# EPFL-VILAB/omnidata

Hardware: AMD Instinct MI355X
Metric: images/sec (384x384) DPT-Hybrid surface-normal inference (higher is better)
Workload: dtype bf16; 1 GPU; DPT-Hybrid-384 normal, batch 32/GPU, bf16, 1xMI355X (BASELINE.json configs[1]); batch_per_gpu=32, global_batch=32, parallelism=replicas x1 (no collective in the loop), ranks_seen=1, inflight=1

## Files before the change

### include/dptx.h

```cpp
#ifndef DPTX_H_
#define DPTX_H_

#include <stddef.h>
#include <stdint.h>

#ifdef __cplusplus
extern "C" {
#endif

typedef struct dptx_engine* dptx_handle;

enum {
  DPTX_OK = 0,
  DPTX_E_INVALID = -1,
  DPTX_E_KEY = -2,
  DPTX_E_HIP = -3,
  DPTX_E_NODEVICE = -4,
  DPTX_E_ALLOC = -5
};

enum { DPTX_DTYPE_BF16 = 0, DPTX_DTYPE_FP16 = 1, DPTX_DTYPE_BF16X3 = 2,
       DPTX_DTYPE_FP16X3 = 3, DPTX_DTYPE_MIXED = 4,
       DPTX_DTYPE_FP8 = 5 };
enum { DPTX_GROUP_RESNET = 1,
// ... 54 lines not shown
int dptx_forward_dual(dptx_handle h, const void* x_dev, int32_t x_dtype, void* y_normal_dev, void* y_depth_dev,
                      int32_t batch, int32_t height, int32_t width, void* stream);

int dptx_set_layer_precision(dptx_handle h, const char* conv_weight_key, int32_t mfmas);

int dptx_calibrate_fp8(dptx_handle h, const void* x_dev, int32_t x_dtype, void* y_dev, void* y2_dev,
                       int32_t batch, int32_t height, int32_t width, void* stream);
int dptx_fp8_get_calibration(dptx_handle h, float* scales, float* amax, int32_t capacity);
int dptx_fp8_set_calibration(dptx_handle h, const float* scales, int32_t n);

int dptx_range_status(dptx_handle h, int32_t* nonfinite, int32_t reset, void* stream);

int dptx_tap(dptx_handle h, const char* name, float* dst_host, size_t capacity_floats,
             int64_t shape4[4]);
int dptx_enable_taps(dptx_handle h, int on);

int dptx_forward_info(dptx_handle h, int64_t* launches, double* algorithmic_macs,
                      double* executed_macs);

int dptx_tune_schedule(dptx_handle h, const void* x_dev, int32_t x_dtype, void* y_dev, void* y_depth_dev, int32_t batch,
                       int32_t height, int32_t width, int32_t reps, void* stream);
int dptx_schedule_info(dptx_handle h, int32_t* split, int32_t* tuned, float* ms_single, float* ms_split);

int dptx_probe_stream_overlap(int32_t device_id, void* stream_a, void* stream_b, int32_t spin_us, float* ratio);

int dptx_set_profiling(dptx_handle h, int on);
int dptx_profile_get(dptx_handle h, int32_t category, double* ms, int64_t* launches,
                     double* macs_per_image);
int dptx_profile_dump(dptx_handle h, const char* path);

const char* dptx_last_error(dptx_handle h);
const char* dptx_version(void);

int dptx_preprocess_u8(const void* img_dev, int32_t H, int32_t W, int32_t C, int32_t row_stride_bytes,
                       int32_t depth_normalize, void* x_dev, void* stream);
int dptx_postprocess_normal_u8(const void* y_dev, void* rgb_u8_dev, void* stream);
int dptx_postprocess_depth(const void* y_dev, void* out512_dev, void* stream);
int dptx_resample_coeffs(int32_t in_size, int32_t out_size, int32_t* bounds, int32_t* kk, int32_t kk_capacity,
                         int32_t* ksize);

int dptx_refocus_workspace_bytes(int32_t B, int32_t C, int32_t H, int32_t W, int32_t n_quantiles, int64_t* bytes);
int dptx_refocus_quantiles(const float* depth, int32_t B, int32_t H, int32_t W, int32_t n_quantiles,
                           float* qvals , void* ws, int64_t ws_bytes, void* stream);
int dptx_refocus(const float* rgb, const float* depth, int32_t B, int32_t C, int32_t H, int32_t W, int32_t n_quantiles,
                 const float* qvals, const float* focus , const float* aperture ,
                 float* out, int64_t* segments , void* ws, int64_t ws_bytes, void* stream);

#define DPTX_MIDAS_SSI 1
#define DPTX_MIDAS_GRAD 2
#define DPTX_MIDAS_ALIGN 4
#define DPTX_MIDAS_INVERSE 8
#define DPTX_MIDAS_ALL 15
#define DPTX_MIDAS_RECORD_DOUBLES 32
#define DPTX_MIDAS_STATS 8
int dptx_midas_workspace_bytes(int32_t B, int32_t H, int32_t W, int32_t scales, int64_t* bytes);
int dptx_midas_loss(const float* pred, const float* target, const uint8_t* mask, int32_t B, int32_t H, int32_t W, int32_t terms,
                    int32_t scales, int32_t image_based, float alpha, float* losses, double* record , void* ws,
                    int64_t ws_bytes, void* stream);
int dptx_midas_loss_backward(const float* pred, const float* target, const uint8_t* mask, int32_t B, int32_t H, int32_t W,
                             int32_t terms, int32_t scales, int32_t image_based, float alpha, const double* record,
                             const float* grad_losses, float* grad_pred, void* stream);
int dptx_midas_stats(const float* pred, const float* target, const uint8_t* mask, int32_t B, int32_t H, int32_t W, int32_t terms,
                     float* stats, float* pred_aligned , float* target_aligned , void* ws,
                     int64_t ws_bytes, void* stream);

#define DPTX_VNL_RECORD_HEADER 64
int dptx_vnl_workspace_bytes(int32_t B, int32_t H, int32_t W, int32_t n, int64_t* bytes);
int dptx_vnl_prepare(const int32_t* p1, const int32_t* p2, const int32_t* p3, int32_t n, int32_t H, int32_t W, uint32_t* inverse,
                     void* ws, int64_t ws_bytes, void* stream);
int dptx_vnl_loss(const float* first, const float* second, int32_t B, int32_t H, int32_t W, float fx, float fy, float delta_z,
                  const int32_t* p1, const int32_t* p2, const int32_t* p3, int32_t n, int32_t select, float* loss_out,
                  uint8_t* record , void* ws, int64_t ws_bytes, void* stream);
int dptx_vnl_loss_backward(const float* first, const float* second, int32_t B, int32_t H, int32_t W, float fx, float fy,
                           const int32_t* p1, const int32_t* p2, const int32_t* p3, int32_t n, const uint8_t* record,
                           const uint32_t* inverse, const float* grad_out, float* grad_first ,
                           float* grad_second , void* stream);
int dptx_vnl_triples(const float* first, const float* second, int32_t B, int32_t H, int32_t W, float fx, float fy, float delta_z,
                     const int32_t* p1, const int32_t* p2, const int32_t* p3, int32_t n, uint8_t* keep, float* loss,
                     float* normals , void* stream);

#define DPTX_NORMAL_L1 1
#define DPTX_NORMAL_COS 2
#define DPTX_NORMAL_CLAMP_PRED 4
#define DPTX_NORMAL_RECORD_DOUBLES 1
int dptx_normal_workspace_bytes(int32_t B, int32_t H, int32_t W, int64_t* bytes);
int dptx_normal_loss(const float* pred, const float* target, const uint8_t* mask, int32_t B, int32_t H, int32_t W, int32_t flags,
                     float l1_weight, float* losses, double* record , void* ws, int64_t ws_bytes, void* stream);
int dptx_normal_loss_backward(const float* pred, const float* target, const uint8_t* mask, int32_t B, int32_t H, int32_t W,
                              int32_t flags, float l1_weight, const double* record, const float* grad_losses, float* grad_pred,
                              void* stream);
int dptx_normal_pixels(const float* pred, const float* target, const uint8_t* mask, int32_t B, int32_t H, int32_t W, int32_t flags,
                       float* cos , float* l1 , void* stream);
#define DPTX_MASKED_L1 0
#define DPTX_MASKED_MSE 1
#define DPTX_MASKED_VALUE 2
#define DPTX_MASKED_EMPTY_ZERO 4
int dptx_masked_workspace_bytes(int64_t n, int64_t* bytes);
int dptx_masked_loss(const float* pred, const float* target , const uint8_t* mask, int64_t n, int32_t kind,
                     float* loss, double* record , void* ws, int64_t ws_bytes, void* stream);
int dptx_masked_loss_backward(const float* pred, const float* target, const uint8_t* mask, int64_t n, int32_t kind,
                              const double* record, const float* grad_loss, float* grad_pred, void* stream);
int dptx_valid_mask(const float* mask_float, int32_t B, int32_t H, int32_t W, int32_t pool, uint8_t* valid, void* stream);

#define DPTX_EVAL_PER_IMAGE 1
#define DPTX_EVAL_NORMAL_FIELDS 9
#define DPTX_EVAL_DEPTH_FIELDS 8
int dptx_eval_workspace_bytes(int32_t B, int32_t H, int32_t W, int64_t* bytes);
int dptx_eval_normal(const float* pred, const float* target , const uint8_t* mask , int32_t B, int32_t H,
                     int32_t W, int32_t flags, double* out , void* ws, int64_t ws_bytes, void* stream);
int dptx_eval_depth(const float* pred, const float* target , const uint8_t* mask , int32_t B, int32_t H,
                    int32_t W, int32_t flags, double* out , void* ws, int64_t ws_bytes, void* stream);
int dptx_eval_normal_pixels(const float* pred, const float* target, int32_t B, int32_t H, int32_t W, double* ang, void* stream);


int dptx_op_set_planes(int64_t act_plane_elems, int64_t w_plane_elems);

int dptx_op_gemm(int32_t dtype, const void* A, const void* W, const float* bias, const void* R,
                 void* C, int32_t M, int32_t N, int32_t K, int32_t act, int32_t a_fp32,
                 int32_t c_fp32, int32_t r_fp32, void* stream);
int dptx_op_conv(int32_t dtype, const void* X, const void* Wt, const float* bias, const void* R,
                 void* Y, int32_t B, int32_t H, int32_t W, int32_t Cin, int32_t Cout,
                 int32_t ksize, int32_t stride, int32_t pad_t, int32_t pad_l, int32_t Ho,
                 int32_t Wo, int32_t a_relu, int32_t act, void* stream);
int dptx_op_conv_planes(int32_t dtype, const void* X, const void* Wt, const float* bias, const void* R, void* Y, int32_t B,
                        int32_t H, int32_t W, int32_t Cin, int32_t Cout, int32_t ksize, int32_t stride, int32_t pad_t,
                        int32_t pad_l, int32_t Ho, int32_t Wo, int32_t a_relu, int32_t act, int32_t epi2, int32_t c_hi_only,
                        int32_t r1_hi_only, void* stream);
int dptx_op_stem_conv(int32_t dtype, const float* x, const void* Wt, void* y, int32_t B, int32_t H, int32_t W,
                      void* stream);
int dptx_op_attention(int32_t dtype, const void* qkv, void* out, int32_t B, int32_t S,
                      int32_t heads, void* stream);
int dptx_op_layernorm(int32_t dtype, const float* x, const float* gamma, const float* beta,
                      void* y, int32_t M, int32_t C, float eps, void* stream);
int dptx_op_groupnorm(int32_t dtype, const void* X, const float* gamma, const float* beta,
                      const void* R, void* Y, int32_t B, int32_t HW, int32_t C, int32_t relu,
                      float eps, void* scratch_f32, void* stream);
int dptx_op_gn_relu_maxpool(int32_t dtype, const void* X, const float* gamma, const float* beta, void* Y, int32_t B,
                            int32_t H, int32_t W, int32_t C, float eps, void* scratch_f32, void* stream);
int dptx_op_cls_rows(int32_t dtype, const float* cls, const float* pos, float* X, int32_t B, int32_t S, int32_t C, void* X16,
                     float* row_stats, void* X8, float q_scale, void* stream);
int dptx_debug_set_trace(void* dev_buf);
int dptx_debug_arena_fill(dptx_handle h, int32_t byte_value);
int dptx_debug_arena_read(dptx_handle h, void* dst_host, size_t offset, size_t bytes);
int dptx_debug_arena_layout(dptx_handle h, char* dst, size_t capacity);
int dptx_debug_arena_checksums(dptx_handle h, void* out_dev, int32_t capacity, void* stream);
int dptx_debug_set_gemm_flags(int32_t flags);
int dptx_op_conv_fp8(const void* X8, const void* Wt8, const float* bias, const void* R, void* Y, void* Y8, int32_t B,
                     int32_t H, int32_t W, int32_t Cin, int32_t Cout, int32_t ksize, int32_t stride, int32_t pad_t,
                     int32_t pad_l, int32_t Ho, int32_t Wo, int32_t act, int32_t q_relu, float out_scale, void* stream);
int dptx_op_conv_groupnorm(int32_t dtype, const void* X, const void* Wt, void* Yraw, const float* gamma, const float* beta,
                           const void* R, void* Y, int32_t B, int32_t H, int32_t W, int32_t Cin, int32_t Cout,
                           int32_t ksize, int32_t stride, int32_t pad_t, int32_t pad_l, int32_t Ho, int32_t Wo,
                           int32_t relu, float eps, void* scratch_f32, void* stream);
int dptx_op_upsample2x(int32_t dtype, const void* X, void* Y, int32_t B, int32_t H, int32_t W,
                       int32_t C, void* stream);
int dptx_op_gemm_ln(int32_t dtype, const void* A, const void* W, const float* bias, void* C, int32_t M, int32_t N, int32_t K,
                    int32_t act, const float* ln_stats, const float* ln_colsum, int32_t ln_nblk, float ln_eps, void* stream);
int dptx_op_gemm_stream(int32_t dtype, const void* A, const void* W, const float* bias, void* C, float* row_stats, int32_t M,
                        int32_t N, int32_t K, void* stream);
int dptx_op_gemm_stream32(int32_t dtype, const void* A, const void* W, const float* bias, float* X, void* C16, float* row_stats,
                          int32_t M, int32_t N, int32_t K, void* stream);
int dptx_op_head_tail(int32_t dtype, const void* H0, const void* W2, const float* b2, const float* w4,
                      const float* b4, float* y, int32_t B, int32_t Hs, int32_t Ws, int32_t C,
                      int32_t relu_out, void* stream);

#ifdef __cplusplus
}
#endif
#endif
```

### omnidata_amd/build.py

```python
from __future__ import annotations

import os
import subprocess
import sys

HERE = os.path.dirname(os.path.abspath(__file__))
CSRC = os.path.join(HERE, "csrc")
LIB = os.path.join(HERE, "libdptx.so")
SOURCES = ["gemm.hip", "gemm_fp16.hip", "gemm_fp16e.hip", "gemm_x3.hip", "gemm_x2.hip", "gemm_fp8.hip", "attention.hip", "norm.hip", "misc.hip", "stem.hip", "head.hip", "prepost.hip", "refocus.hip", "midas_loss.hip", "vnl_loss.hip", "normal_loss.hip", "eval_metrics.hip", "engine.hip", "ops.hip"]
HEADERS = ["common.h", "kernels.h", "gemm_impl.h", "select.h", os.path.join("..", "..", "include", "dptx.h")]
_NOPK = ["-Xclang", "-target-feature", "-Xclang", "-packed-fp32-ops"]
SOURCE_FLAGS = {src: list(_NOPK) for src in ("norm.hip", "misc.hip", "gemm.hip", "gemm_fp16.hip", "gemm_fp16e.hip", "gemm_x3.hip",
                                             "gemm_x2.hip", "gemm_fp8.hip", "refocus.hip",
                                             "midas_loss.hip", "vnl_loss.hip", "normal_loss.hip", "eval_metrics.hip")}
EXPERIMENT_HEADERS = []


def source_hash(extra_flags=()) -> str:
    import hashlib
    h = hashlib.sha256()
    for name in sorted(SOURCES + HEADERS + EXPERIMENT_HEADERS):
        path = os.path.join(CSRC, name)
        h.update(os.path.basename(name).encode() + b"\0")
        with open(path, "rb") as f:
            h.update(f.read())
    h.update(" ".join(extra_flags).encode())
    h.update(repr(sorted(SOURCE_FLAGS.items())).encode())
    return h.hexdigest()[:16]


def _newer(dst: str, srcs) -> bool:
    if not os.path.exists(dst):
        return False
    t = os.path.getmtime(dst)
    return all(os.path.getmtime(s) <= t for s in srcs)


def built_hash(suffix: str = "") -> str:
    path = os.path.join(CSRC, "build" + suffix, "engine.srchash")
    return open(path).read().strip() if os.path.exists(path) else ""


def build(force: bool = False, verbose: bool = False) -> str:
    import fcntl
    suffix = os.environ.get("DPTX_LIB_SUFFIX", "")
    objdir = os.path.join(CSRC, "build" + suffix)
    os.makedirs(objdir, exist_ok=True)
    with open(os.path.join(objdir, ".lock"), "w") as lock:
        fcntl.flock(lock, fcntl.LOCK_EX)
        try:
            return _build_locked(force, verbose, suffix, objdir)
        finally:
            fcntl.flock(lock, fcntl.LOCK_UN)


def _build_locked(force: bool, verbose: bool, suffix: str, objdir: str) -> str:
    hipcc = os.environ.get("HIPCC", "/opt/rocm/bin/hipcc")
    extra = os.environ.get("DPTX_CXXFLAGS", "").split()
    LIB = os.path.join(HERE, f"libdptx{suffix}.so")
    hdrs = [os.path.join(CSRC, h) for h in HEADERS + EXPERIMENT_HEADERS]
    src_hash = source_hash(extra)
    hash_file = os.path.join(objdir, "engine.srchash")
    old_hash = open(hash_file).read().strip() if os.path.exists(hash_file) else ""
    objs = []
    procs = []
    for src in SOURCES:
        s = os.path.join(CSRC, src)
        o = os.path.join(objdir, src.replace(".hip", ".o"))
        objs.append(o)
        cmd = [hipcc, "--offload-arch=gfx950", "-O3", "-std=c++17", "-fPIC"] + SOURCE_FLAGS.get(src, []) + extra + ["-c", s, "-o", o]
        if src == "engine.hip":
            cmd.insert(-4, f'-DDPTX_SRC_HASH="{src_hash}"')
        cmd_file = o + ".cmd"
        same_cmd = os.path.exists(cmd_file) and open(cmd_file).read() == " ".join(cmd)
        if not force and same_cmd and _newer(o, [s] + hdrs):
            continue
        if verbose:
            print(" ".join(cmd))
        if os.path.exists(cmd_file):
            os.remove(cmd_file)
        procs.append((src, cmd_file, " ".join(cmd), subprocess.Popen(cmd, stdout=subprocess.PIPE, stderr=subprocess.STDOUT, text=True)))
    for src, cmd_file, cmd_txt, p in procs:
        out, _ = p.communicate()
        if p.returncode != 0:
            raise RuntimeError(f"hipcc failed on {src}:\n{out}")
        with open(cmd_file, "w") as f:
            f.write(cmd_txt)
    if force or procs or not _newer(LIB, objs):
        tmp = f"{LIB}.tmp{os.getpid()}"
        cmd = [hipcc, "--offload-arch=gfx950", "-shared", "-fPIC", "-o", tmp] + objs
        r = subprocess.run(cmd, stdout=subprocess.PIPE, stderr=subprocess.STDOUT, text=True)
        if r.returncode != 0:
            if os.path.exists(tmp):
                os.remove(tmp)
            raise RuntimeError(f"link failed:\n{r.stdout}")
        os.replace(tmp, LIB)
    with open(hash_file, "w") as f:
        f.write(src_hash + "\n")
    return LIB


if __name__ == "__main__":
    print(build(force="--force" in sys.argv, verbose=True))
```

### omnidata_amd/csrc/engine.hip

```cpp
#include <hip/hip_runtime.h>

#include <algorithm>
#include <cmath>
#include <cstdio>
#include <chrono>
#include <cstring>
#include <map>
#include <memory>
#include <string>
#include <unordered_map>
#include <vector>

#include "../../include/dptx.h"
#include "kernels.h"

using namespace dptx;

namespace {

constexpr int IMG = 384;
constexpr int S_TOK = 577;
constexpr int FEAT = 256;
const int STAGE_DEPTH[3] = {3, 4, 9};
const int STAGE_OUT[3] = {256, 512, 1024};
// ... 488 lines not shown
      const uint16_t hi = f32_to_fp16(x);
      d16[i] = hi;
      if (x3) d16[i + lo_elems] = f32_to_fp16(x - fp16_to_f32(hi));
      return;
    }
    const uint16_t hi = f32_to_bf16(x);
    d16[i] = hi;
    if (x3) d16[i + lo_elems] = f32_to_bf16(x - bf16_to_f32(hi));
  };
  auto r16 = [&](float x) { return bf ? bf16_to_f32(f32_to_bf16(x)) : fp16_to_f32(f32_to_fp16(x)); };
  for (const auto& s : e->spec) {
    if (s.role == R_UNUSED || s.role == R_DERIVED) continue;
    const std::vector<float>& src = e->staged.at(s.key);
    uint8_t* dst = e->host_blob.data() + e->packed_off.at(s.key);
    const bool fold_w = e->ln_fold && s.role == R_LINEAR && (ends_with(s.key, "attn.qkv.weight") || ends_with(s.key, "mlp.fc1.weight"));
    const bool fold_b = e->ln_fold && s.role == R_VEC && (ends_with(s.key, "attn.qkv.bias") || ends_with(s.key, "mlp.fc1.bias"));
    if (fold_w || fold_b) {
      const bool qkv = s.key.find("attn.qkv") != std::string::npos;
      const std::string blk = s.key.substr(0, s.key.find(qkv ? "attn.qkv" : "mlp.fc1"));
      const std::string wkey = blk + (qkv ? "attn.qkv.weight" : "mlp.fc1.weight");
      const std::vector<float>& W = e->staged.at(wkey);
      const std::vector<float>& gamma = e->staged.at(blk + (qkv ? "norm1.weight" : "norm2.weight"));
      const std::vector<float>& beta = e->staged.at(blk + (qkv ? "norm1.bias" : "norm2.bias"));
      const size_t K = gamma.size(), N = W.size() / K;
      if (fold_b) {
        float* d32 = (float*)dst;
        for (size_t n = 0; n < N; ++n) {
          double acc = src[n];
          for (size_t k = 0; k < K; ++k) acc += (double)W[n * K + k] * (double)beta[k];
          d32[n] = (float)acc;
        }
      } else {
        uint16_t* d16 = (uint16_t*)dst;
        float* cs = (float*)(e->host_blob.data() + e->packed_off.at(blk + (qkv ? "attn.qkv.lnsum" : "mlp.fc1.lnsum")));
        for (size_t n = 0; n < N; ++n) {
          double acc = 0.0;
          for (size_t k = 0; k < K; ++k) {
            const float wf = W[n * K + k] * gamma[k];
            put(d16, n * K + k, wf);
            acc += (double)r16(wf);
          }
          cs[n] = (float)acc;
        }
      }
      continue;
    }
    if (s.role == R_VEC || s.role == R_HEAD4) {
      memcpy(dst, src.data(), src.size() * 4);
      continue;
    }
    if (s.role == R_DECONV_BIAS) {
      for (int t = 0; t < 16; ++t) memcpy(dst + (size_t)t * src.size() * 4, src.data(), src.size() * 4);
      continue;
    }
    uint16_t* d16 = (uint16_t*)dst;
    if (s.role == R_LINEAR) {
      for (size_t i = 0; i < src.size(); ++i) put(d16, i, src[i]);
      continue;
    }
    if (s.role == R_DECONV) {
      const int CI = (int)s.shape[0], CO = (int)s.shape[1], K = (int)s.shape[2];
      for (int ci = 0; ci < CI; ++ci)
        for (int co = 0; co < CO; ++co)
          for (int dy = 0; dy < K; ++dy)
            for (int dx = 0; dx < K; ++dx)
              put(d16, ((size_t)(dy * K + dx) * CO + co) * CI + ci, src[(((size_t)ci * CO + co) * K + dy) * K + dx]);
      continue;
    }
    const int O = (int)s.shape[0], I = (int)s.shape[1], KH = (int)s.shape[2], KW = (int)s.shape[3];
    const size_t per_o = (size_t)I * KH * KW;
    const bool stem = (KH == 7);
    const size_t out_k = stem ? STEM_K : per_o;
    for (int o = 0; o < O; ++o) {
      const float* wo = src.data() + (size_t)o * per_o;
      double mean = 0.0, scale = 1.0;
      if (s.role == R_STDCONV) {
        double sum = 0.0;
        for (size_t i = 0; i < per_o; ++i) sum += wo[i];
        mean = sum / (double)per_o;
        double var = 0.0;
        for (size_t i = 0; i < per_o; ++i) { const double t = wo[i] - mean; var += t * t; }
        var /= (double)per_o;
        scale = e->cfg.ws_form == 0 ? 1.0 / (std::sqrt(var) + (double)e->cfg.ws_eps)
                                    : 1.0 / std::sqrt(var + (double)e->cfg.ws_eps);
      }
      for (int ky = 0; ky < KH; ++ky)
        for (int kx = 0; kx < KW; ++kx)
          for (int i = 0; i < I; ++i) {
            const double wv = ((double)wo[((size_t)i * KH + ky) * KW + kx] - mean) * scale;
            const size_t kidx = stem ? ((size_t)i * 7 + ky) * 8 + kx : ((size_t)ky * KW + kx) * I + i;
            put(d16, (size_t)o * out_k + kidx, (float)wv);
          }
    }
  }
  if (e->fp8()) {
    for (size_t si = 0; si < e->spec.size(); ++si) {
      const Spec& sp = e->spec[si];
      if (sp.role != R_CONV || !dptx_engine::fp8_weight(sp.key)) continue;
      const size_t off = e->packed_off.at(sp.key);
      const std::vector<float>& src = e->staged.at(sp.key);
      const int O = (int)sp.shape[0], I = (int)sp.shape[1], KH = (int)sp.shape[2], KW = (int)sp.shape[3];
      const size_t per_o = (size_t)I * KH * KW;
      uint8_t* d8 = e->host_blob.data() + e->packed_single + off / 2;
      float* inv = (float*)(e->host_blob.data() + e->packed_off.at(sp.key.substr(0, sp.key.size() - 6) + "f8scale"));
      for (int o = 0; o < O; ++o) {
        float mx = 0.f;
        for (size_t i = 0; i < per_o; ++i) mx = std::max(mx, std::fabs(src[(size_t)o * per_o + i]));
        const float sc = e4m3_channel_scale(mx, &inv[o]);
        for (int ky = 0; ky < KH; ++ky)
          for (int kx = 0; kx < KW; ++kx)
            for (int i = 0; i < I; ++i)
              d8[(size_t)o * per_o + ((size_t)ky * KW + kx) * I + i] = f32_to_e4m3(src[(((size_t)o * I + i) * KH + ky) * KW + kx] * sc);
      }
    }
  }
  if (e->fp8()) {
    for (size_t si = 0; si < e->spec.size(); ++si) {
      const Spec& sp = e->spec[si];
      if (sp.role != R_LINEAR || !dptx_engine::fp8_vit_weight(sp.key)) continue;
      const std::vector<float>& W = e->staged.at(sp.key);
      const size_t N = (size_t)sp.shape[0], K = (size_t)sp.shape[1];
      const bool fc2 = ends_with(sp.key, "mlp.fc2.weight"), qkv = ends_with(sp.key, "attn.qkv.weight");
      const std::string stem_key = sp.key.substr(0, sp.key.size() - 6);
      const std::string blk = sp.key.substr(0, sp.key.find(qkv ? "attn.qkv" : (fc2 ? "mlp.fc2" : "mlp.fc1")));
      const std::vector<float>* gamma = (!fc2 && e->ln_fold) ? &e->staged.at(blk + (qkv ? "norm1.weight" : "norm2.weight")) : nullptr;
      uint8_t* d8 = e->host_blob.data() + e->packed_single + e->packed_off.at(sp.key) / 2;
      float* inv = (float*)(e->host_blob.data() + e->packed_off.at(stem_key + "f8scale"));
      float* cs8 = fc2 ? nullptr : (float*)(e->host_blob.data() + e->packed_off.at(stem_key + "lnsum8"));
      for (size_t n = 0; n < N; ++n) {
        float mx = 0.f;
        for (size_t k = 0; k < K; ++k) mx = std::max(mx, std::fabs(W[n * K + k] * (gamma ? (*gamma)[k] : 1.0f)));
        const float sc = e4m3_channel_scale(mx, &inv[n]);
        double acc = 0.0;
        for (size_t k = 0; k < K; ++k) {
          const uint8_t q = f32_to_e4m3(W[n * K + k] * (gamma ? (*gamma)[k] : 1.0f) * sc);
          d8[n * K + k] = q;
          acc += (double)e4m3_to_f32(q);
        }
        if (cs8) cs8[n] = (float)(acc / (double)sc);
      }
    }
  }
  e->finalized = true;
  return DPTX_OK;
}

enum { LN_NONE = 0, LN_CONSUMER = 1, LN_PRODUCER = 2 };
struct GemmOpt {
  const float* bias_ = nullptr;
  int act_ = 0, a_relu_ = 0;
  const void *R1_ = nullptr, *R2_ = nullptr;
  int q_ = 0;
  float* gn_part_ = nullptr;
  int out_lo_ = -1;
  int c_fp32_ = 0, r1_fp32_ = 0;
  int ln_ = LN_NONE;
  const float* colsum_ = nullptr;
  GemmOpt& bias(const float* v) { bias_ = v; return *this; }
  GemmOpt& act(int v) { act_ = v; return *this; }
  GemmOpt& a_relu(int v) { a_relu_ = v; return *this; }
  GemmOpt& R1(const void* v) { R1_ = v; return *this; }
  GemmOpt& R2(const void* v) { R2_ = v; return *this; }
  GemmOpt& q(int v) { q_ = v; return *this; }
  GemmOpt& gn_part(float* v) { gn_part_ = v; return *this; }
  GemmOpt& out_lo(int v) { out_lo_ = v; return *this; }
  GemmOpt& c_fp32(int v) { c_fp32_ = v; return *this; }
  GemmOpt& r1_fp32(int v) { r1_fp32_ = v; return *this; }
  GemmOpt& ln(int v) { ln_ = v; return *this; }
  GemmOpt& colsum(const float* v) { colsum_ = v; return *this; }
};

struct Run {
  dptx_engine* e;
  int B;
  hipStream_t st;
  int dt;
  int Hi = 384, Wi = 384;
  int io = 0;
  size_t abase = 0;
  bool half = false;
  hipError_t err = hipSuccess;
  const char* where = "";
  int64_t launches = 0;
  double exec_macs = 0.0, cat_macs[4] = {0, 0, 0, 0};
  std::unordered_map<const void*, int> q8_slot;
  int q8_count = 0;
  int q8_produce(const void* out) {
    const int slot = q8_count < dptx_engine::MAX_Q8 ? q8_count : dptx_engine::MAX_Q8 - 1;
    ++q8_count;
    q8_slot[out] = slot;
    return slot;
  }
  float q8_scale_of(const void* in) const {
    auto it = q8_slot.find(in);
    return it == q8_slot.end() ? 1.0f : e->act_scale[it->second];
  }
  void q8_measure(const void* out, size_t n, int relu, int slot) {
    if (e->calibrating && e->d_amax) chk(launch_amax(MODE_BF16, out, n, relu, e->d_amax + slot, st), "fp8.amax");
  }

  char* A(const Buf& b) const { return e->d_arena + abase + (half ? b.off2 : b.off); }

  void chk(hipError_t r, const char* w, int cat = 3) {
    if (err == hipSuccess && r != hipSuccess) { err = r; where = w; }
    launches++;
    if (e->profiling) {
      const size_t i = e->event_cat.size() + 1;
      if (i >= e->events.size()) {
        hipEvent_t ev;
        if (hipEventCreate(&ev) != hipSuccess) return;
        e->events.push_back(ev);
      }
      (void)hipEventRecord(e->events[i], st);
      e->event_cat.push_back(cat);
      e->event_name.emplace_back(w);
    }
  }
  void gemm(int mode, const GemmParams& p, const char* name) {
    exec_macs += (double)p.M / B * p.N * p.K;
    cat_macs[0] += (double)p.M / B * p.N * p.K;
    chk(launch_gemm(mode, p, st), name, 0);
  }
  std::unordered_map<const void*, bool> lo_valid_;
  bool has_lo(const void* p) const {
    auto it = lo_valid_.find(p);
    return it != lo_valid_.end() && it->second;
  }
  void mark_lo(const void* p, bool v) { lo_valid_[p] = v; }
  int cur_group = 0;
  void tap(const char* name, const void* p, int64_t h, int64_t w, int64_t c, bool fp32 = false) {
    int m = dt;
    if (e->mixed() && lo_valid_.count(p)) m = has_lo(p) ? MODE_FP16X3 : MODE_FP16;
    e->taps[name] = TapInfo{p, {B, h, w, c}, fp32, m};
  }
  void group(int g) { dt = e->mode_of(g); cur_group = g; }

  void conv(const void* in, int Hin, int Win, int Cin, const std::string& wkey, int ksz, int stride, int pad_t, int pad_l,
            int Hout, int Wout, int Cout, void* out, const GemmOpt& o = GemmOpt()) {
    const bool f8 = e->fp8_use(wkey) && !e->calibrating;
    GemmParams p;
    gemm_params_conv(p, B, Hin, Win, Cin, Cout, ksz, stride, pad_t, pad_l, Hout, Wout, f8 ? 1 : 2);
    p.A = in; p.W = e->w(wkey); p.C = out; p.bias = o.bias_; p.R1 = o.R1_; p.R2 = o.R2_;
    int slot = -1;
    if (e->fp8() && o.q_) {
      slot = q8_produce(out);
      p.C8 = e->q8(out); p.q_relu = o.q_ == 2; p.q_scale = e->act_scale[slot];
    }
    p.act = o.act_; p.a_relu = o.a_relu_; p.planes = e->pl;
    if (o.gn_part_) { p.gn_part = o.gn_part_; p.gn_hw = Hout * Wout; p.gn_blocks = Hout * Wout / 32; p.gn_cpg = Cout / 32; }
    if (f8) {
      p.A = e->q8(in); p.W = e->w8(wkey); p.a_relu = 0;
      p.out_scale = 1.0f / q8_scale_of(in); p.out_scale_v = e->wscale(wkey);
    }
    int mode = f8 ? MODE_FP8 : dt;
    if (o.out_lo_ >= 0 && e->mixed()) {
      const bool x3 = e->layer_x3(wkey, cur_group), a_lo = e->layer_reads_lo(wkey, cur_group);
      p.a_hi_only = x3 && !a_lo;
      if (a_lo && !has_lo(in)) {
        if (err == hipSuccess) { err = hipErrorInvalidValue; where = "precision policy: a 3-MFMA layer reads a tensor without lo plane"; }
        return;
      }
      const bool r1lo = o.R1_ != nullptr && has_lo(o.R1_), r2lo = o.R2_ != nullptr && has_lo(o.R2_);
      mode = x3 ? MODE_FP16X3 : MODE_FP16;
      p.r1_hi_only = !r1lo; p.r2_hi_only = !r2lo; p.c_hi_only = !o.out_lo_;
      p.epi2 = (!x3 && (o.out_lo_ || r1lo || r2lo)) ? 1 : 0;
      mark_lo(out, o.out_lo_ != 0);
    }
    gemm(mode, p, wkey.c_str());
    if (slot >= 0) q8_measure(out, (size_t)p.M * p.N, o.q_ == 2, slot);
  }

  static bool gn_fusable(int HW) { return HW % 32 == 0; }
  void gn_stats(const void* X, float* part, int HW, int C) { chk(launch_gn_stats(dt, X, part, B, HW, C, e->pl, st), "gn_stats", 2); }
  void gn_apply(void* X, const std::string& nkey, float* part, int HW, int C, int relu, const void* R = nullptr,
                const std::string& rkey = "", const float* rpart = nullptr) {
    GnParams g{};
    g.nrec = gn_fusable(HW) ? HW / 32 : 0;
    g.X = X; g.Y = X; g.gamma = e->f(nkey + ".weight"); g.beta = e->f(nkey + ".bias"); g.partial = part;
    g.R = R;
    if (!rkey.empty()) { g.r_gamma = e->f(rkey + ".weight"); g.r_beta = e->f(rkey + ".bias"); g.r_partial = rpart; }
    g.B = B; g.HW = HW; g.C = C; g.relu = relu; g.eps = 1e-5f;
    chk(launch_gn_apply(dt, g, e->pl, st), nkey.c_str(), 2);
  }

  void rcu(const std::string& p, const void* x, int H, int W, void* tmp, void* out, const GemmOpt& o) {
    const int mid_lo = e->mixed() ? (int)e->layer_reads_lo(p + "conv2.weight", cur_group) : -1;
    conv(x, H, W, FEAT, p + "conv1.weight", 3, 1, 1, 1, H, W, FEAT, tmp,
         GemmOpt().bias(e->f(p + "conv1.bias")).act(1).a_relu(1).q(e->fp8_use(p + "conv2.weight") ? 1 : 0).out_lo(mid_lo));
    conv(tmp, H, W, FEAT, p + "conv2.weight", 3, 1, 1, 1, H, W, FEAT, out,
         GemmOpt().bias(e->f(p + "conv2.bias")).R1(x).R2(o.R2_).q(o.q_).out_lo(e->mixed() ? o.out_lo_ : -1));
  }

  int forward(const void* x, void* y, void* y2);
};

int Run::forward(const void* x, void* y, void* y2) {
  dptx_engine* E = e;
  E->taps.clear();
  E->event_cat.clear();
  E->event_name.clear();
  if (E->profiling) {
    if (E->events.empty()) {
      hipEvent_t ev;
      if (hipEventCreate(&ev) == hipSuccess) E->events.push_back(ev);
    }
    if (!E->events.empty()) (void)hipEventRecord(E->events[0], st);
  }
  const std::string vp = "pretrained.model.";
  const std::string bp = vp + "patch_embed.backbone.";
  const int D_VIT = E->dv, D_MLP = E->dm, N_HEADS = E->nh;
  const bool large = E->backbone == DPTX_BACKBONE_VITL16_384;
  float* part0 = (float*)A(E->part[0]);
  float* part1 = (float*)A(E->part[1]);
  float* part2 = (float*)A(E->part[2]);
  float* part3 = (float*)A(E->part[3]);
  const int h2 = Hi / 2, w2 = Wi / 2, h4 = Hi / 4, w4 = Wi / 4, gh = Hi / 16, gw = Wi / 16, h32 = Hi / 32, w32 = Wi / 32;
  const int NP = gh * gw;
  const int S = NP + 1;
  const bool native = (gh == 24 && gw == 24);
  const float* pos = E->f("pretrained.model.pos_embed");
  if (!native) {
    chk(launch_pos_resize(pos, (float*)A(E->pos_alt), 24, gh, gw, D_VIT, st), "pos_resize");
    pos = (const float*)A(E->pos_alt);
  }

  if (!large) {
  group(DPTX_GROUP_RESNET);
  chk(launch_stem_conv(dt, x, io, E->w(bp + "stem.conv.weight"), A(E->sraw), B, Hi, Wi, E->pl, st), "stem.conv", 0);
  exec_macs += (double)h2 * w2 * 64 * STEM_K;
  cat_macs[0] += (double)h2 * w2 * 64 * STEM_K;
  gn_stats(A(E->sraw), part0, h2 * w2, 64);
  chk(launch_gn_relu_maxpool(dt, A(E->sraw), A(E->stem), E->f(bp + "stem.norm.weight"), E->f(bp + "stem.norm.bias"),
                             part0, B, h2, w2, 64, 1e-5f, E->pl, st),
      "stem.pool", 2);
  tap("stem", A(E->stem), h4, w4, 64);

  const void* cur = A(E->stem);
  int H = h4, Wd = w4, cin = 64;
  for (int s = 0; s < 3; ++s) {
    const int cout = STAGE_OUT[s], mid = cout / 4;
    for (int b = 0; b < STAGE_DEPTH[s]; ++b) {
      const std::string p = bp + "stages." + std::to_string(s) + ".blocks." + std::to_string(b) + ".";
      const int stride = (b == 0) ? STAGE_STRIDE[s] : 1;
      const int Ho = H / stride, Wo = Wd / stride;
      void* out = (b == STAGE_DEPTH[s] - 1) ? (void*)A(E->S[s]) : (void*)((b & 1) ? A(E->PB) : A(E->PA));
      const bool f_in = gn_fusable(H * Wd), f_out = gn_fusable(Ho * Wo);
      if (b == 0) {
        conv(cur, H, Wd, cin, p + "downsample.conv.weight", 1, stride, 0, 0, Ho, Wo, cout, A(E->DS), GemmOpt().gn_part(f_out ? part3 : nullptr));
        if (!f_out) gn_stats(A(E->DS), part3, Ho * Wo, cout);
      }
      conv(cur, H, Wd, cin, p + "conv1.weight", 1, 1, 0, 0, H, Wd, mid, A(E->T1), GemmOpt().gn_part(f_in ? part0 : nullptr));
      if (!f_in) gn_stats(A(E->T1), part0, H * Wd, mid);
      gn_apply(A(E->T1), p + "norm1", part0, H * Wd, mid, 1);
      const int pad = (stride == 1) ? 1 : 0;
      conv(A(E->T1), H, Wd, mid, p + "conv2.weight", 3, stride, pad, pad, Ho, Wo, mid, A(E->T2), GemmOpt().gn_part(f_out ? part1 : nullptr));
      if (!f_out) gn_stats(A(E->T2), part1, Ho * Wo, mid);
      gn_apply(A(E->T2), p + "norm2", part1, Ho * Wo, mid, 1);
      conv(A(E->T2), Ho, Wo, mid, p + "conv3.weight", 1, 1, 0, 0, Ho, Wo, cout, out, GemmOpt().gn_part(f_out ? part2 : nullptr));
      if (!f_out) gn_stats(out, part2, Ho * Wo, cout);
      if (b == 0)
        gn_apply(out, p + "norm3", part2, Ho * Wo, cout, 1, A(E->DS), p + "downsample.norm", part3);
      else
        gn_apply(out, p + "norm3", part2, Ho * Wo, cout, 1, cur);
      cur = out;
      H = Ho;
      Wd = Wo;
      cin = cout;
    }
    const char* names[3] = {"s0", "s1", "s2"};
    tap(names[s], cur, H, Wd, cout);
  }
  }

  float* X = (float*)A(E->X);
  float* lnst = (float*)A(E->lnst);
  const int ln_nblk = D_VIT / 128;
  const bool s16 = E->stream16;
  group(DPTX_GROUP_EMBED);
  int hn_slot = -1;
  {
    const int Kp = large ? 768 : 1024;
    if (large) chk(launch_patchify16(dt, x, io, A(E->F1), B, Hi, Wi, E->pl, st), "patchify");
    GemmParams p;
    gemm_params_dense(p, B * NP, D_VIT, Kp);
    p.A = large ? A(E->F1) : A(E->S[2]); p.W = E->w(vp + "patch_embed.proj.weight"); p.C = X;
    p.bias = E->f(vp + "patch_embed.proj.bias");
    p.c_rpi = NP; p.c_img_rows = S; p.c_row_off = 1; p.ldc = D_VIT; p.c_fp32 = 1;
    p.R2 = pos; p.r2_bcast = 1; p.r2_fp32 = 1; p.planes = E->pl;
    if (E->ln_fold) { p.C16 = A(E->Hn); p.row_stats = lnst; p.stats_nblk = 8; }
    if (s16) { p.C = A(E->Hn); p.c_fp32 = 0; p.C16 = nullptr; }
    hn_slot = E->fp8_use(vp + "blocks.0.attn.qkv.weight") ? q8_produce(A(E->Hn)) : -1;
    if (hn_slot >= 0) { p.C8 = E->q8(A(E->Hn)); p.q_relu = 0; p.q_scale = E->act_scale[hn_slot]; }
    gemm(dt, p, "patch_embed.proj");
  }
  chk(launch_cls_rows(E->mode_of(DPTX_GROUP_VIT), E->f(vp + "cls_token"), pos, s16 ? nullptr : X, B, S, D_VIT,
                      E->ln_fold ? A(E->Hn) : nullptr, E->ln_fold ? lnst : nullptr, st,
                      hn_slot >= 0 ? E->q8(A(E->Hn)) : nullptr, hn_slot >= 0 ? E->act_scale[hn_slot] : 1.0f),
      "cls_rows");
  if (hn_slot >= 0) q8_measure(A(E->Hn), (size_t)B * S * D_VIT, 0, hn_slot);
  const int M = B * S;
  const size_t tok_elems = (size_t)M * D_VIT;
  auto tok_tap = [&](int idx, const char* name) {
    if (!E->taps_on) return;
    float* dst = E->d_tok_taps + (size_t)idx * E->tok_tap_stride;
    if (s16) {
      const hipError_t r = launch_to_f32(E->mode_of(DPTX_GROUP_VIT), A(E->Hn), dst, tok_elems, E->pl, st);
      if (err == hipSuccess && r != hipSuccess) { err = r; where = "tok_tap"; }
    } else if (err == hipSuccess) {
      err = hipMemcpyAsync(dst, X, tok_elems * 4, hipMemcpyDeviceToDevice, st);
    }
    E->taps[name] = TapInfo{dst, {B, S, D_VIT, 1}, true, dt};
  };
  tok_tap(0, "tok0");

  auto dense = [&](const void* A, const std::string& wkey, int N, int K, void* C, const GemmOpt& o) {
    GemmParams p;
    gemm_params_dense(p, M, N, K);
    p.A = A; p.W = E->w(wkey); p.C = C; p.c_fp32 = o.c_fp32_; p.bias = o.bias_; p.act = o.act_;
    p.R1 = o.R1_; p.r1_fp32 = o.r1_fp32_; p.planes = E->pl;
    if (o.ln_ == LN_CONSUMER) { p.ln_stats = lnst; p.ln_colsum = o.colsum_; p.ln_nblk = ln_nblk; p.ln_eps = 1e-6f; p.ln_inv_dim = 1.0f / (float)K; }
    if (o.ln_ == LN_PRODUCER) { p.C16 = this->A(E->Hn); p.row_stats = lnst; p.stats_nblk = 8; }
    if (o.ln_ == LN_PRODUCER && s16) {
      p.C = this->A(E->Hn); p.c_fp32 = 0; p.R1 = this->A(E->Hn); p.r1_fp32 = 0; p.C16 = nullptr;
    }
    int mode = dt;
    if (E->fp8_use(wkey) && !E->calibrating) {
      p.A = E->q8(A); p.W = E->w8(wkey); p.a_bytes /= 2;
      p.out_scale = 1.0f / q8_scale_of(A); p.out_scale_v = E->wscale(wkey);
      if (o.ln_ == LN_CONSUMER) p.ln_colsum = E->f(wkey.substr(0, wkey.size() - 6) + "lnsum8");
      mode = MODE_FP8;
    }
    int slot = -1;
    if (o.q_) {
      slot = q8_produce(p.C);
      p.C8 = E->q8(p.C); p.q_relu = 0; p.q_scale = E->act_scale[slot];
    }
    gemm(mode, p, wkey.c_str());
    if (slot >= 0) q8_measure(p.C, (size_t)M * N, 0, slot);
  };

  auto readout = [&](int n) {
    group(DPTX_GROUP_REASSEMBLE);
    const std::string pp = "pretrained.act_postprocess" + std::to_string(n) + ".";
    float* clsb = (float*)A(E->clsb);
    chk(launch_readout_cls(dt, s16 ? (const float*)A(E->Hn) : X, (long long)S * D_VIT, E->w(pp + "0.project.0.weight"), 2 * D_VIT,
                           D_VIT, E->f(pp + "0.project.0.bias"), clsb, B, D_VIT, D_VIT, E->pl, st, s16 ? 1 : 0),
        "readout_cls");
    if (!(E->ln_fold && !mode_is_x3(dt))) chk(launch_cast_f32(dt, X, A(E->Hn), (size_t)B * S * D_VIT, E->pl, st), "readout_cast");
    exec_macs += (double)D_VIT * D_VIT;
    void* R = (n & 1) ? A(E->R3) : A(E->R4);
    GemmParams p{};
    p.A = A(E->Hn); p.a_bytes = (long long)B * S * D_VIT * 2; p.planes = E->pl;
    p.W = E->w(pp + "0.project.0.weight"); p.ldw = 2 * D_VIT; p.C = R;
    p.M = B * NP; p.N = D_VIT; p.K = D_VIT;
    p.a_rpi = NP; p.Wout = NP; p.Hin = 1; p.Win = NP; p.Cin = D_VIT; p.a_pix_stride = D_VIT;
    p.a_img_stride = (long long)S * D_VIT; p.a_off = D_VIT;
    p.ksz = 1; p.stride = 1;
    p.c_rpi = NP; p.c_img_rows = NP; p.c_row_off = 0; p.ldc = D_VIT;
    p.bias = clsb; p.bias_per_img = 1; p.act = 2;
    gemm(dt, p, "readout");
    const int f = n == 1 ? 256 : (n == 2 ? 512 : D_VIT);
    conv(R, gh, gw, D_VIT, pp + "3.weight", 1, 1, 0, 0, gh, gw, f, n == 3 ? A(E->L3) : A(E->T4), GemmOpt().bias(E->f(pp + "3.bias")));
    if (n <= 2) {
      const int k = n == 1 ? 4 : 2;
      GemmParams d;
      gemm_params_dense(d, B * NP, k * k * f, f);
      d.A = A(E->T4); d.W = E->w(pp + "4.weight"); d.C = A(E->F1); d.bias = E->f(pp + "4.bias"); d.planes = E->pl;
      gemm(dt, d, "reassemble.deconv");
      chk(launch_depth_to_space(dt, A(E->F1), A(E->S[n - 1]), B, gh, gw, k, f, E->pl, st), "reassemble.d2s");
      tap(n == 1 ? "l1" : "l2", A(E->S[n - 1]), gh * k, gw * k, f);
    } else if (n == 3) {
      tap("l3", A(E->L3), gh, gw, D_VIT);
    } else {
      conv(A(E->T4), gh, gw, D_VIT, pp + "4.weight", 3, 2, 1, 1, h32, w32, D_VIT, A(E->L4), GemmOpt().bias(E->f(pp + "4.bias")));
      tap("l4", A(E->L4), h32, w32, D_VIT);
    }
  };

  for (int l = 0; l < E->depth; ++l) {
    group(DPTX_GROUP_VIT);
    const std::string p = vp + "blocks." + std::to_string(l) + ".";
    const bool lf = E->ln_fold;
    const int ln_in = lf ? LN_CONSUMER : LN_NONE, ln_out = lf ? LN_PRODUCER : LN_NONE;
    if (!lf) chk(launch_layernorm(dt, X, E->f(p + "norm1.weight"), E->f(p + "norm1.bias"), A(E->Hn), M, D_VIT, 1e-6f, E->pl, st), "ln1", 2);
    const std::string pn = vp + "blocks." + std::to_string(l + 1) + ".";
    const bool q_fc1 = E->fp8_use(p + "mlp.fc1.weight"), q_fc2 = E->fp8_use(p + "mlp.fc2.weight");
    const bool q_next = l + 1 < E->depth && E->fp8_use(pn + "attn.qkv.weight");
    dense(A(E->Hn), p + "attn.qkv.weight", 3 * D_VIT, D_VIT, A(E->QKV),
          GemmOpt().bias(E->f(p + "attn.qkv.bias")).ln(ln_in).colsum(E->f(p + "attn.qkv.lnsum")));
    chk(launch_attention(dt, A(E->QKV), A(E->AO), B, S, N_HEADS, E->pl, st), "attention", 1);
    exec_macs += 2.0 * N_HEADS * (double)S * S * 64;
    cat_macs[1] += 2.0 * N_HEADS * (double)S * S * 64;
    dense(A(E->AO), p + "attn.proj.weight", D_VIT, D_VIT, X,
          GemmOpt().c_fp32(1).bias(E->f(p + "attn.proj.bias")).R1(X).r1_fp32(1).ln(ln_out).q(q_fc1));
    if (!lf) chk(launch_layernorm(dt, X, E->f(p + "norm2.weight"), E->f(p + "norm2.bias"), A(E->Hn), M, D_VIT, 1e-6f, E->pl, st), "ln2", 2);
    dense(A(E->Hn), p + "mlp.fc1.weight", D_MLP, D_VIT, A(E->F1),
          GemmOpt().bias(E->f(p + "mlp.fc1.bias")).act(2).ln(ln_in).colsum(E->f(p + "mlp.fc1.lnsum")).q(q_fc2));
    dense(A(E->F1), p + "mlp.fc2.weight", D_VIT, D_MLP, X,
          GemmOpt().c_fp32(1).bias(E->f(p + "mlp.fc2.bias")).R1(X).r1_fp32(1).ln(ln_out).q(q_next));
    {
      char nm[16];
      snprintf(nm, sizeof nm, "blk%d", l);
      tok_tap(l + 1, nm);
    }
    if (large) {
      if (l % 6 == 5) readout(l / 6 + 1);
    } else {
      if (l == 8) readout(3);
      if (l == 11) readout(4);
    }
  }
// ... 780 lines not shown
```

### omnidata_amd/csrc/gemm.hip

```cpp
#include "gemm_impl.h"

namespace dptx {

hipError_t launch_gemm_16(int dt, const GemmParams& p, hipStream_t stream) {
  return dt == DT_BF16 ? launch_dt<DT_BF16, 1>(p, stream) : launch_gemm_fp16(p, stream);
}

void gemm_params_dense(GemmParams& p, int M, int N, int K) {
  p = GemmParams{};
  p.M = M; p.N = N; p.K = K; p.ldw = K;
  p.a_rpi = M > 0 ? M : 1; p.Wout = p.a_rpi; p.Hin = 1; p.Win = p.a_rpi; p.Cin = K; p.a_pix_stride = K;
  p.a_img_stride = 0; p.a_off = 0; p.ksz = 1; p.stride = 1; p.pad_t = 0; p.pad_l = 0;
  p.c_rpi = 0x7fffffff; p.c_img_rows = 0; p.c_row_off = 0; p.ldc = N;
  p.a_bytes = (long long)M * K * 2;
}

void gemm_params_conv(GemmParams& p, int B, int Hin, int Win, int Cin, int Cout, int ksz, int stride, int pad_t, int pad_l,
                      int Hout, int Wout, int a_elem_bytes) {
  p = GemmParams{};
  p.M = B * Hout * Wout; p.N = Cout; p.K = ksz * ksz * Cin; p.ldw = p.K;
  p.a_rpi = Hout * Wout; p.Wout = Wout; p.Hin = Hin; p.Win = Win; p.Cin = Cin; p.a_pix_stride = Cin;
  p.a_img_stride = (long long)Hin * Win * Cin; p.a_off = 0; p.ksz = ksz; p.stride = stride; p.pad_t = pad_t; p.pad_l = pad_l;
  p.c_rpi = 0x7fffffff; p.c_img_rows = 0; p.c_row_off = 0; p.ldc = Cout;
  p.a_bytes = (long long)B * Hin * Win * Cin * a_elem_bytes;
  p.k_tap_fast = (ksz == 3 && Cin >= 512) ? 1 : 0;
}

static thread_local long long* g_trace = nullptr;
void gemm_set_trace(long long* dev_buf) { g_trace = dev_buf; }
static thread_local int g_debug_flags = 0;
void gemm_set_debug_flags(int flags) { g_debug_flags = flags; }
static thread_local float g_cu_share = 1.0f;
void gemm_set_cu_share(float share) { g_cu_share = share > 0.f && share <= 1.f ? share : 1.0f; }

hipError_t launch_gemm(int mode, const GemmParams& p0, hipStream_t stream) {
  GemmParams p = p0;
  p.trace = g_trace;
  p.debug_flags = g_debug_flags;
  if (p.cu_share <= 0.f) p.cu_share = g_cu_share;
  p.a_rpi_rcp = 1.0f / (float)(p.a_rpi > 0 ? p.a_rpi : 1);
  p.wout_rcp = 1.0f / (float)(p.Wout > 0 ? p.Wout : 1);
  if (p.gn_part != nullptr && (p.gn_hw % 32 != 0 || p.N % 32 != 0 || p.gn_cpg != p.N / 32 || p.gn_cpg < 2 || p.gn_cpg > 32 ||
                               (p.gn_cpg & (p.gn_cpg - 1)) != 0 || p.bias != nullptr || p.act != 0))
    return hipErrorInvalidValue;
  if (p.row_stats != nullptr && (p.N % 128 != 0 || p.stats_nblk != 8 || p.N / 128 > 8)) return hipErrorInvalidValue;
  if (p.ln_stats != nullptr && (p.R1 != nullptr || p.R2 != nullptr || p.bias_per_img || p.ln_colsum == nullptr || (p.ln_nblk != 6 && p.ln_nblk != 8) ||
                                p.c_rpi != 0x7fffffff || p.gn_part != nullptr))
    return hipErrorInvalidValue;
  if (mode == MODE_FP8) {
    if (p.K % 128 != 0 || p.Cin % 128 != 0 || p.M <= 0 || p.N % 32 != 0 || p.ldw < p.K || p.ldw % 16 != 0 || p.gn_part != nullptr)
      return hipErrorInvalidValue;
    return launch_gemm_fp8(p, stream);
  }
  if (p.K % BK != 0 || p.Cin % BK != 0 || p.M <= 0 || p.N % 32 != 0 || p.ldw < p.K || p.ldw % 8 != 0) return hipErrorInvalidValue;
  if (mode == MODE_BF16) return p.epi2 ? hipErrorInvalidValue : launch_gemm_16(DT_BF16, p, stream);
  if (mode == MODE_FP16) return p.epi2 ? launch_gemm_fp16e(p, stream) : launch_gemm_16(DT_FP16, p, stream);
  if (mode == MODE_BF16X3) return launch_gemm_x3(DT_BF16, p, stream);
  if (mode == MODE_FP16X3) return p.a_hi_only ? launch_gemm_x2(p, stream) : launch_gemm_x3(DT_FP16, p, stream);
  return hipErrorInvalidValue;
}

}
```

### omnidata_amd/csrc/gemm_impl.h

```cpp
#pragma once
#include <cstdlib>
#include <type_traits>

#include "common.h"
#include "kernels.h"

namespace dptx {

constexpr int BK = 64;

__device__ __forceinline__ int row_div(int m, int d, float rcp, bool big, int& rem) {
  if (big) {
    const int q = m / d;
    rem = m - q * d;
    return q;
  }
  int q = (int)((float)m * rcp);
  int r = m - q * d;
  if (r < 0) { --q; r += d; }
  if (r >= d) { ++q; r -= d; }
  rem = r;
  return q;
}

__device__ __forceinline__ float2 ln_mu_rstd(float sm, float sq, float inv_dim, float eps) {
  const float mu = sm * inv_dim;
  const float var = (float)((double)sq * (double)inv_dim - (double)mu * (double)mu);
  return make_float2(mu, __builtin_amdgcn_rsqf(fmaxf(var, 0.f) + eps));
}

__device__ __forceinline__ float ln_fold_fma(float acc, float mu, float rstd, float colsum, float bias) {
  float t = fmaf(-mu, colsum, acc);
  asm volatile("" : "+v"(t));
  t = fmaf(t, rstd, bias);
  asm volatile("" : "+v"(t));
  return t;
}

template <int DT, int TM, int TN, bool RELU_A, int PL = 1, int HK = BK / 16, int XT = 3>
__device__ __forceinline__ void mma_tile(const char* sa, const char* sb, int a_lo, int b_lo, int wm, int wn, int lr, int lh,
                                         f32x16_t (&acc)[TM][TN]) {
  if constexpr (DT == DT_FP8) {
    static_assert(PL == 1 && !RELU_A, "fp8: single plane; the producer writes the ReLU'd copy");
    typedef int i32x8_t __attribute__((ext_vector_type(8)));
#pragma unroll
    for (int q = 0; q < 2; ++q) {
      i32x8_t af[TM], bf[TN];
      const int c0 = 4 * q + 2 * lh;
#pragma unroll
      for (int i = 0; i < TM; ++i) {
        const int row = wm * (TM * 32) + i * 32 + lr;
        const int sw = (row >> 1) & 7;
        const u32x4_t lo = *(const u32x4_t*)(sa + row * 128 + ((c0 ^ sw) << 4));
        const u32x4_t hi = *(const u32x4_t*)(sa + row * 128 + (((c0 + 1) ^ sw) << 4));
        af[i] = i32x8_t{(int)lo.x, (int)lo.y, (int)lo.z, (int)lo.w, (int)hi.x, (int)hi.y, (int)hi.z, (int)hi.w};
      }
#pragma unroll
      for (int j = 0; j < TN; ++j) {
        const int row = wn * (TN * 32) + j * 32 + lr;
        const int sw = (row >> 1) & 7;
        const u32x4_t lo = *(const u32x4_t*)(sb + row * 128 + ((c0 ^ sw) << 4));
        const u32x4_t hi = *(const u32x4_t*)(sb + row * 128 + (((c0 + 1) ^ sw) << 4));
        bf[j] = i32x8_t{(int)lo.x, (int)lo.y, (int)lo.z, (int)lo.w, (int)hi.x, (int)hi.y, (int)hi.z, (int)hi.w};
      }
#pragma unroll
      for (int i = 0; i < TM; ++i)
#pragma unroll
        for (int j = 0; j < TN; ++j)
          acc[i][j] = __builtin_amdgcn_mfma_scale_f32_32x32x64_f8f6f4(af[i], bf[j], acc[i][j], 0, 0, 0, 0x7f7f7f7f, 0, 0x7f7f7f7f);
    }
    return;
  } else if constexpr (PL == 1) {
#pragma unroll
    for (int g = 0; g < BK / 16; g += HK) {
      u32x4_t af[HK][TM], bf[HK][TN];
#pragma unroll
      for (int ks = 0; ks < HK; ++ks) {
        const int chunk = 2 * (g + ks) + lh;
#pragma unroll
        for (int i = 0; i < TM; ++i) {
          const int row = wm * (TM * 32) + i * 32 + lr;
          af[ks][i] = *(const u32x4_t*)(sa + row * 128 + ((chunk ^ ((row >> 1) & 7)) << 4));
        }
#pragma unroll
        for (int j = 0; j < TN; ++j) {
          const int row = wn * (TN * 32) + j * 32 + lr;
          bf[ks][j] = *(const u32x4_t*)(sb + row * 128 + ((chunk ^ ((row >> 1) & 7)) << 4));
        }
      }
      __builtin_amdgcn_sched_barrier(0);
#pragma unroll
      for (int ks = 0; ks < HK; ++ks) {
#pragma unroll
        for (int i = 0; i < TM; ++i) {
          if (RELU_A) af[ks][i] = relu8(af[ks][i]);
#pragma unroll
          for (int j = 0; j < TN; ++j) acc[i][j] = T16<DT>::mfma32(af[ks][i], bf[ks][j], acc[i][j]);
        }
      }
      if (HK != BK / 16) __builtin_amdgcn_sched_barrier(0);
    }
    return;
  } else {
    u32x4_t af[2][TM], bf[2][TN], al[2][TM], bl[2][TN];
    auto read = [&](int s_, int ks) {
      const int chunk = 2 * ks + lh;
#pragma unroll
      for (int i = 0; i < TM; ++i) {
        const int row = wm * (TM * 32) + i * 32 + lr;
        const int off = row * 128 + ((chunk ^ ((row >> 1) & 7)) << 4);
        af[s_][i] = *(const u32x4_t*)(sa + off);
        if (XT == 3) al[s_][i] = *(const u32x4_t*)(sa + a_lo + off);
      }
#pragma unroll
      for (int j = 0; j < TN; ++j) {
        const int row = wn * (TN * 32) + j * 32 + lr;
        const int off = row * 128 + ((chunk ^ ((row >> 1) & 7)) << 4);
        bf[s_][j] = *(const u32x4_t*)(sb + off);
        bl[s_][j] = *(const u32x4_t*)(sb + b_lo + off);
      }
    };
    auto mma = [&](int s_) {
#pragma unroll
      for (int i = 0; i < TM; ++i) {
        if (RELU_A) {
          if (XT == 3) relu8_planes(af[s_][i], al[s_][i]);
          else af[s_][i] = relu8(af[s_][i]);
        }
#pragma unroll
        for (int j = 0; j < TN; ++j) {
          if (XT == 3) acc[i][j] = T16<DT>::mfma32(al[s_][i], bf[s_][j], acc[i][j]);
          acc[i][j] = T16<DT>::mfma32(af[s_][i], bl[s_][j], acc[i][j]);
          acc[i][j] = T16<DT>::mfma32(af[s_][i], bf[s_][j], acc[i][j]);
        }
      }
    };
    read(0, 0);
#pragma unroll
    for (int ks = 0; ks < BK / 16; ++ks) {
      if (ks + 1 < BK / 16) read((ks + 1) & 1, ks + 1);
      __builtin_amdgcn_sched_barrier(0);
      mma(ks & 1);
      __builtin_amdgcn_sched_barrier(0);
    }
  }
}

template <int DT, int BM, int BN, int TM, int TN, int PL = 1, int NT = 256, int SLABS = 1, bool WP = false>
__device__ __forceinline__ void epilogue(const GemmParams& p, char* smem, int m0, int n0, int wm, int wn, int lr, int lh,
                                         int tid, f32x16_t (&acc)[TM][TN], int row_pitch = 0, bool dma_in_flight = false,
                                         int trace_row = -1, const char* lds_ln = nullptr) {
  static_assert(SLABS == 1 || SLABS == TM, "one slab, or one per MFMA row tile");
  static_assert(!WP || (SLABS == TM && TN == 2), "wave-private staging: one 32 x 64 block per wave and slab");
  constexpr int CT_PITCH = WP ? 72 : BN + 4;
  constexpr int CT_ROWS = WP ? 32 : BM / SLABS;
  constexpr int NCH = WP ? 8 : BN / 8;
  constexpr int RPP = WP ? 8 : NT / NCH;
  constexpr int ITER = CT_ROWS / RPP;
  constexpr int WAVES_N = BN / (TN * 32);
  static_assert(CT_ROWS % RPP == 0, "rows per pass must divide the slab");
#ifdef DPTX_TRACE
#define DPTX_ESTAMP(SLOT)                                                                                          \
  do {                                                                                                             \
    if (p.trace != nullptr && blockIdx.x == 0 && tid == 0 && trace_row >= 0)                                       \
      p.trace[(48 + trace_row) * 4 + (SLOT)] = (long long)__builtin_readcyclecounter();                            \
  } while (0)
#else
#define DPTX_ESTAMP(SLOT) do { } while (0)
  (void)trace_row;
#endif
  DPTX_ESTAMP(0);
  float* ct = (float*)smem + (WP ? (wm * WAVES_N + wn) * (32 * CT_PITCH) : 0);
  const int cn = WP ? tid & 7 : tid % NCH;
  const int rr = WP ? (tid & 63) >> 3 : tid / NCH;
  const int n = n0 + (WP ? wn * (TN * 32) : 0) + cn * 8;

  if (p.gn_part != nullptr) {
    const int cpg = p.gn_cpg;
    const int cpg_sh = __builtin_ctz(cpg);
    int gn_hw = p.gn_hw;
    asm volatile("" : "+s"(gn_hw));
#pragma unroll
    for (int i = 0; i < TM; ++i) {
      const int mb = m0 + (wm * TM + i) * 32;
      const int img = mb / gn_hw;
      const int blk = (mb - img * gn_hw) >> 5;
#pragma unroll
      for (int j = 0; j < TN; ++j) {
        float sm = 0.f, sq = 0.f;
#pragma unroll
        for (int r = 0; r < 16; ++r) { const float v = acc[i][j][r]; sm += v; sq = fmaf(v, v, sq); }
        sm += __shfl_xor(sm, 32, 64);
        sq += __shfl_xor(sq, 32, 64);
        for (int o = 1; o < cpg; o <<= 1) { sm += __shfl_xor(sm, o, 64); sq += __shfl_xor(sq, o, 64); }
        if (lh == 0 && (lr & (cpg - 1)) == 0 && mb < p.M) {
          const int g = (n0 + (wn * TN + j) * 32 + lr) >> cpg_sh;
          float2* dst = (float2*)p.gn_part + ((long long)img * p.gn_blocks + blk) * 32 + g;
          *dst = make_float2(sm, sq);
        }
      }
    }
  }

  float bias_c[8];
#pragma unroll
  for (int e = 0; e < 8; ++e) bias_c[e] = 0.f;
  if (p.bias != nullptr && !p.bias_per_img) {
    const float4 b0 = *(const float4*)(p.bias + n), b1 = *(const float4*)(p.bias + n + 4);
    bias_c[0] = b0.x; bias_c[1] = b0.y; bias_c[2] = b0.z; bias_c[3] = b0.w;
    bias_c[4] = b1.x; bias_c[5] = b1.y; bias_c[6] = b1.z; bias_c[7] = b1.w;
  }
  float osc[8];
  if (p.out_scale != 0.f) {
#pragma unroll
    for (int e = 0; e < 8; ++e) osc[e] = p.out_scale;
    if (p.out_scale_v != nullptr) {
      const float4 s0 = *(const float4*)(p.out_scale_v + n), s1 = *(const float4*)(p.out_scale_v + n + 4);
      osc[0] *= s0.x; osc[1] *= s0.y; osc[2] *= s0.z; osc[3] *= s0.w;
      osc[4] *= s1.x; osc[5] *= s1.y; osc[6] *= s1.z; osc[7] *= s1.w;
    }
  }
  const bool remap = p.c_rpi != 0x7fffffff;
  int c_rpi = p.c_rpi;
  asm volatile("" : "+s"(c_rpi));
  float2* lnrow = (float2*)(smem + (WP ? (size_t)(NT / 64) * 32 * CT_PITCH * 4 : (size_t)CT_ROWS * CT_PITCH * 4));
  if (p.ln_stats != nullptr) {
    const bool all8 = p.ln_nblk == 8;
    for (int r = tid; r < BM; r += NT) {
      int R = r;
      if (row_pitch) R = (R >> 5) * row_pitch + (R & 31);
      int m = m0 + R;
      m = m < p.M ? m : m0;
      const float4* st = lds_ln != nullptr ? (const float4*)(lds_ln + r * 64) : (const float4*)(p.ln_stats + (long long)m * 16);
      const float4 r0 = st[0], r1_ = st[1], r2_ = st[2], r3_ = st[3];
      const float sm = (r0.x + r0.z) + (r1_.x + r1_.z) + ((r2_.x + r2_.z) + (all8 ? r3_.x + r3_.z : 0.f));
      const float sq = (r0.y + r0.w) + (r1_.y + r1_.w) + ((r2_.y + r2_.w) + (all8 ? r3_.y + r3_.w : 0.f));
      lnrow[r] = ln_mu_rstd(sm, sq, p.ln_inv_dim, p.ln_eps);
    }
    if (WP) __syncthreads();
  }
  DPTX_ESTAMP(1);
  constexpr int GR_ = SLABS > 1 ? 2 : (ITER < 4 ? ITER : 4);
  static_assert(ITER % GR_ == 0, "row groups");

  auto body = [&](auto r1m_, auto r2m_, auto bpi_, auto lnf_) {
    constexpr int R1M = decltype(r1m_)::value, R2M = decltype(r2m_)::value, BPI = decltype(bpi_)::value;
    constexpr bool LNF = decltype(lnf_)::value != 0;
    constexpr int GR = (SLABS > 1 && (R1M < 0 || (PL == 2 && R1M != 0 && R2M != 0))) ? 1 : GR_;
// ... 52 lines not shown
            rb[it][0] = src[0];
            rb[it][1] = src[1];
          } else {
            rb[it][0] = *(const u32x4_t*)((const uint16_t*)p.R2 + off);
            if (PL == 2) {
              rb[it][1] = u32x4_t{0u, 0u, 0u, 0u};
              if (!p.r2_hi_only) rb[it][1] = *(const u32x4_t*)((const uint16_t*)p.R2 + p.planes.act + off);
            }
          }
        }
        if (bpi) {
          const u32x4_t* src = (const u32x4_t*)(p.bias + (long long)img * p.N + n);
          bb[it][0] = src[0];
          bb[it][1] = src[1];
        }
      }
    };
#pragma unroll
    for (int s = 0; s < SLABS; ++s) {
      issue_loads(s, 0);
      if (WP) __builtin_amdgcn_wave_barrier();
      else if (s > 0) __syncthreads();
#pragma unroll
      for (int i = 0; i < TM; ++i) {
        if (SLABS != 1 && i != s) continue;
#pragma unroll
        for (int j = 0; j < TN; ++j)
#pragma unroll
          for (int r = 0; r < 16; ++r) {
            const int ml = (WP ? 0 : SLABS == 1 ? wm * (TM * 32) + i * 32 : wm * 32) + (r & 3) + 8 * (r >> 2) + 4 * lh;
            const int nl = (WP ? j * 32 : wn * (TN * 32) + j * 32) + lr;
            ct[ml * CT_PITCH + nl] = acc[i][j][r];
          }
      }
      if (s == 0 && dma_in_flight) asm volatile("s_waitcnt vmcnt(0)" ::: "memory");
      if (WP) __builtin_amdgcn_wave_barrier();
      else __syncthreads();
#pragma unroll
      for (int gi = 0; gi < NGR; ++gi) {
        if (gi > 0) issue_loads(s, gi);
#pragma unroll
        for (int it = 0; it < GR; ++it) {
          const int row = rr + (gi * GR + it) * RPP;
          float v[8];
          {
            const float4 x0 = *(const float4*)(ct + row * CT_PITCH + cn * 8);
            const float4 x1 = *(const float4*)(ct + row * CT_PITCH + cn * 8 + 4);
            v[0] = x0.x; v[1] = x0.y; v[2] = x0.z; v[3] = x0.w;
            v[4] = x1.x; v[5] = x1.y; v[6] = x1.z; v[7] = x1.w;
          }
          if (p.out_scale != 0.f) {
#pragma unroll
            for (int e = 0; e < 8; ++e) v[e] *= osc[e];
          }
          if (LNF) {
            const float2 ms = lnrow[ln_R[it]];
#ifdef DPTX_LN_PACKED_FMA
#pragma unroll
            for (int e = 0; e < 8; ++e) v[e] = fmaf(fmaf(-ms.x, ln_c[e], v[e]), ms.y, bias_c[e]);
#else
#pragma unroll
            for (int e = 0; e < 8; ++e) v[e] = ln_fold_fma(v[e], ms.x, ms.y, ln_c[e], bias_c[e]);
#endif
          } else if (bpi) {
#pragma unroll
            for (int e = 0; e < 4; ++e) { v[e] += __uint_as_float(bb[it][0][e]); v[4 + e] += __uint_as_float(bb[it][1][e]); }
          } else {
#pragma unroll
            for (int e = 0; e < 8; ++e) v[e] += bias_c[e];
          }
          if (p.act == 1) {
#pragma unroll
            for (int e = 0; e < 8; ++e) v[e] = fmaxf(v[e], 0.f);
          } else if (p.act == 2) {
#pragma unroll
            for (int e = 0; e < 8; e += 2) gelu_erf2(v[e], v[e + 1]);
          }
          if (r1) {
            if (r1f) {
#pragma unroll
              for (int e = 0; e < 4; ++e) { v[e] += __uint_as_float(ra[it][0][e]); v[4 + e] += __uint_as_float(ra[it][1][e]); }
            } else {
              float f[8];
              unpack8x<DT, PL>(ra[it][0], ra[it][1], f);
#pragma unroll
              for (int e = 0; e < 8; ++e) v[e] += f[e];
            }
          }
          if (r2) {
            if (r2f) {
#pragma unroll
              for (int e = 0; e < 4; ++e) { v[e] += __uint_as_float(rb[it][0][e]); v[4 + e] += __uint_as_float(rb[it][1][e]); }
            } else {
              float f[8];
              unpack8x<DT, PL>(rb[it][0], rb[it][1], f);
#pragma unroll
              for (int e = 0; e < 8; ++e) v[e] += f[e];
            }
          }
          if (p.row_stats != nullptr) {
            float sm = 0.f, sq = 0.f;
#pragma unroll
            for (int e = 0; e < 8; ++e) { sm += v[e]; sq = fmaf(v[e], v[e], sq); }
#pragma unroll
            for (int o = 1; o < 16; o <<= 1) { sm += __shfl_xor(sm, o, 64); sq += __shfl_xor(sq, o, 64); }
            if (ok[it] && (cn & 15) == 0)
              ((float2*)p.row_stats)[(long long)crow_[it] * p.stats_nblk + ((n0 + cn * 8) >> 7)] = make_float2(sm, sq);
          }
          if (ok[it]) {
            if (p.C16 != nullptr) store8f<DT, 1>((uint16_t*)p.C16 + coff[it], 0, v);
            if (p.c_fp32) {
              float* cp = (float*)p.C + coff[it];
              *(float4*)cp = make_float4(v[0], v[1], v[2], v[3]);
              *(float4*)(cp + 4) = make_float4(v[4], v[5], v[6], v[7]);
            } else if (PL == 2 && p.c_hi_only) {
              store8f<DT, 1>((uint16_t*)p.C + coff[it], 0, v);
            } else {
              store8f<DT, PL>((uint16_t*)p.C + coff[it], p.planes.act, v);
            }
            if (p.C8 != nullptr) {
              const float qs = p.q_scale != 0.f ? p.q_scale : 1.0f;
              if (p.q_relu) {
#pragma unroll
                for (int e = 0; e < 8; ++e) v[e] = fmaxf(v[e], 0.f);
              }
#pragma unroll
              for (int e = 0; e < 8; ++e) v[e] *= qs;
              *(uint2*)((uint8_t*)p.C8 + coff[it]) = pack_fp8x8(v);
            }
          }
        }
      }
      if (s == 0) DPTX_ESTAMP(2);
    }
    DPTX_ESTAMP(3);
  };
  using std::integral_constant;
  typedef integral_constant<int, 0> I0;
  typedef integral_constant<int, 1> I1;
  typedef integral_constant<int, 2> I2;
  typedef integral_constant<int, -1> IX;
  const bool has1 = p.R1 != nullptr, has2 = p.R2 != nullptr;
  if (p.ln_stats != nullptr) body(I0{}, I0{}, I0{}, I1{});
  else if (!has1 && !has2 && !p.bias_per_img) body(I0{}, I0{}, I0{}, I0{});
  else if (has1 && p.r1_fp32 && !has2 && !p.bias_per_img) body(I2{}, I0{}, I0{}, I0{});
  else if (has1 && !p.r1_fp32 && !has2 && !p.bias_per_img) body(I1{}, I0{}, I0{}, I0{});
  else if (has1 && !p.r1_fp32 && has2 && !p.r2_fp32 && !p.bias_per_img) body(I1{}, I1{}, I0{}, I0{});
  else body(IX{}, IX{}, IX{}, I0{});
#undef DPTX_ESTAMP
}

constexpr unsigned OOB = 0x80000000u;

template <int DT, int BM, int BN, int WAVES_M, int WAVES_N, bool RELU_A, int PL, int PLE = PL, int XT = 3>
__global__ __launch_bounds__(64 * WAVES_M * WAVES_N, PL == 2 ? 1 : 2) void gemm_glds_kernel(const GemmParams p) {
#if defined(__HIP_DEVICE_COMPILE__)
  constexpr int NT = 64 * WAVES_M * WAVES_N;
  static_assert(NT == 256 || NT == 512, "4 or 8 waves per block");
  constexpr int TM = BM / WAVES_M / 32, TN = BN / WAVES_N / 32;
  constexpr int ROWS_PP = NT / 8;
  constexpr int PASS_BYTES = ROWS_PP * 128;
  constexpr int A_PASSES = BM / ROWS_PP, B_PASSES = BN / ROWS_PP;
  constexpr int HK = (TM * TN > 4) ? 2 : BK / 16;
  constexpr int ES = DT == DT_FP8 ? 1 : 2;
  constexpr int KE = 128 / ES;
  constexpr int DTS = DT == DT_FP8 ? DT_BF16 : DT;
  constexpr int SLABS = (BM * (BN + 4) * 4 > 160 * 1024) ? TM : 1;
  constexpr int A_LO = BM * 128, B_BASE = PL * BM * 128, B_LO = BN * 128;
  constexpr int STAGE_BYTES = PL * (BM + BN) * 128;
  extern __shared__ __attribute__((aligned(16))) char smem[];

  const int tid = threadIdx.x;
  const int lane = tid & 63;
  const int wave = __builtin_amdgcn_readfirstlane(tid >> 6);
  const int wm = wave / WAVES_N, wn = wave % WAVES_N;
  const int lr = lane & 31, lh = lane >> 5;

  const int tiles_n = p.N / BN, tiles_m = (p.M + BM - 1) / BM;
  int m0, n0;
  {
    const int x = (int)blockIdx.x & 7, l = (int)blockIdx.x >> 3;
    const int tn_per = tiles_n / p.xcd_n, tm_per = (tiles_m + p.xcd_m - 1) / p.xcd_m;
    const int mt = (x / p.xcd_n) * tm_per + l / tn_per;
    const int nt = (x % p.xcd_n) * tn_per + l % tn_per;
    if (mt >= tiles_m || l >= tm_per * tn_per) return;
    m0 = mt * BM;
    n0 = nt * BN;
  }

  const int kc = tid & 7, r0 = tid >> 3;
  const int sc = kc ^ ((r0 >> 1) & 7);
  int a_iy0[A_PASSES], a_ix0[A_PASSES];
  unsigned a_off[A_PASSES];
#pragma unroll
  for (int i = 0; i < A_PASSES; ++i) {
    const int m = m0 + r0 + ROWS_PP * i;
    const bool ok = m < p.M;
    const int mm = ok ? m : 0;
    int rem, ox;
    const int img = row_div(mm, p.a_rpi, p.a_rpi_rcp, false, rem);
    const int oy = row_div(rem, p.Wout, p.wout_rcp, false, ox);
    a_iy0[i] = ok ? oy * p.stride - p.pad_t : -0x40000000;
    a_ix0[i] = ox * p.stride - p.pad_l;
    const long long e = (long long)img * p.a_img_stride + p.a_off +
                        ((long long)a_iy0[i] * p.Win + a_ix0[i]) * p.a_pix_stride + sc * (16 / ES);
    a_off[i] = (unsigned)(ok ? e * ES : 0);
  }
  unsigned w_off[B_PASSES];
#pragma unroll
  for (int j = 0; j < B_PASSES; ++j) w_off[j] = (unsigned)(((long long)(n0 + r0 + ROWS_PP * j) * p.ldw + sc * (16 / ES)) * ES);

  const int w_bytes = (int)((long long)p.N * p.ldw * ES);
  const __amdgpu_buffer_rsrc_t rsrcA = __builtin_amdgcn_make_buffer_rsrc(const_cast<void*>(p.A), 0, (int)p.a_bytes, 0x00020000);
  const __amdgpu_buffer_rsrc_t rsrcW = __builtin_amdgcn_make_buffer_rsrc(const_cast<void*>(p.W), 0, w_bytes, 0x00020000);
  const __amdgpu_buffer_rsrc_t rsrcAl = __builtin_amdgcn_make_buffer_rsrc(
      (void*)((uint16_t*)const_cast<void*>(p.A) + (PL == 2 ? p.planes.act : 0)), 0, (int)p.a_bytes, 0x00020000);
  const __amdgpu_buffer_rsrc_t rsrcWl = __builtin_amdgcn_make_buffer_rsrc(
      (void*)((uint16_t*)const_cast<void*>(p.W) + (PL == 2 ? p.planes.w : 0)), 0, w_bytes, 0x00020000);

  int ky = 0, kx = 0, c0 = 0;

#define DPTX_ISSUE_TILE(BUF, K0)                                                                                   \
  do {                                                                                                             \
    char* sa_ = smem + (BUF) * STAGE_BYTES + wave * 1024;                                                          \
    char* sb_ = sa_ + B_BASE;                                                                                      \
    const unsigned tap_ = (unsigned)(((ky * p.Win + kx) * p.a_pix_stride + c0) * ES);                              \
    const unsigned wk_ = (unsigned)((((ky * p.ksz + kx) * p.Cin) + c0) * ES);            \
    _Pragma("unroll") for (int i = 0; i < A_PASSES; ++i) {                                                         \
      const int iy = a_iy0[i] + ky, ix = a_ix0[i] + kx;                                                            \
      const bool valid = ((unsigned)iy < (unsigned)p.Hin) && ((unsigned)ix < (unsigned)p.Win);                     \
      const unsigned vo = valid ? a_off[i] + tap_ : OOB;                                                           \
      __builtin_amdgcn_raw_ptr_buffer_load_lds(rsrcA, (__attribute__((address_space(3))) void*)(sa_ + i * PASS_BYTES), 16, vo, 0, \
                                               0, 0);                                                              \
      if (PL == 2 && XT == 3)                                                                                      \
        __builtin_amdgcn_raw_ptr_buffer_load_lds(rsrcAl, (__attribute__((address_space(3))) void*)(sa_ + A_LO + i * PASS_BYTES), \
                                                 16, vo, 0, 0, 0);                                                 \
    }                                                                                                              \
    _Pragma("unroll") for (int j = 0; j < B_PASSES; ++j) {                                                         \
      __builtin_amdgcn_raw_ptr_buffer_load_lds(rsrcW, (__attribute__((address_space(3))) void*)(sb_ + j * PASS_BYTES), 16,   \
                                               w_off[j] + wk_, 0, 0, 0);                                           \
      if (PL == 2)                                                                                                 \
        __builtin_amdgcn_raw_ptr_buffer_load_lds(rsrcWl, (__attribute__((address_space(3))) void*)(sb_ + B_LO + j * PASS_BYTES), \
                                                 16, w_off[j] + wk_, 0, 0, 0);                                     \
    }                                                                                                              \
    if (p.k_tap_fast) {  \
      if (++kx == p.ksz) {                                                                                         \
        kx = 0;                                                                                                    \
        if (++ky == p.ksz) { ky = 0; c0 += KE; }                                                                   \
      }                                                                                                            \
    } else {                                                                    \
      c0 += KE;                                                                                                    \
      if (c0 >= p.Cin) {                                                                                           \
        c0 = 0;                                                                                                    \
        if (++kx == p.ksz) { kx = 0; ++ky; }                                                                       \
      }                                                                                                            \
    }                                                                                                              \
  } while (0)

  f32x16_t acc[TM][TN];
#pragma unroll
  for (int i = 0; i < TM; ++i)
#pragma unroll
    for (int j = 0; j < TN; ++j)
#pragma unroll
      for (int r = 0; r < 16; ++r) acc[i][j][r] = 0.f;

  const int nk = p.K / KE;
  const bool tr = p.trace != nullptr && blockIdx.x == 0 && lane == 0;
  long long* trp = p.trace + wave * 4 * 64;
#ifdef DPTX_TRACE
#define DPTX_STAMP(SLOT) do { if (tr && kt < 64) trp[kt * 4 + (SLOT)] = (long long)__builtin_readcyclecounter(); } while (0)
#else
#define DPTX_STAMP(SLOT) do { } while (0)
#endif
#ifdef DPTX_TRACE
  if (tr && wave == 0) { trp[62 * 4 + 0] = (long long)__builtin_readcyclecounter(); trp[62 * 4 + 1] = (long long)wall_clock64(); }
#endif
  DPTX_ISSUE_TILE(0, 0);
  for (int kt = 0; kt < nk; ++kt) {
    asm volatile("s_waitcnt vmcnt(0)" ::: "memory");
    DPTX_STAMP(3);
    __syncthreads();
    DPTX_STAMP(0);
    const char* sa = smem + (kt & 1) * STAGE_BYTES;
    if (kt + 1 < nk) DPTX_ISSUE_TILE((kt + 1) & 1, (kt + 1) * BK);
    DPTX_STAMP(1);
    mma_tile<DT, TM, TN, RELU_A, PL, HK, XT>(sa, sa + B_BASE, A_LO, B_LO, wm, wn, lr, lh, acc);
    DPTX_STAMP(2);
  }
#ifdef DPTX_TRACE
  if (tr && wave == 0) { trp[62 * 4 + 2] = (long long)__builtin_readcyclecounter(); trp[62 * 4 + 3] = (long long)wall_clock64(); }
#endif
#undef DPTX_STAMP
#undef DPTX_ISSUE_TILE
  __syncthreads();
  epilogue<DTS, BM, BN, TM, TN, PLE, NT, SLABS>(p, smem, m0, n0, wm, wn, lr, lh, tid, acc);
#endif
}

struct PpFrags { u32x4_t a[4], b[2]; };
__device__ __forceinline__ void pp_read(PpFrags& f, const char* sa, const char* sb, int wn, int lr, int lh, int ks) {
  const int chunk = 2 * ks + lh;
#pragma unroll
  for (int i = 0; i < 4; ++i) {
    const int row = i * 32 + lr;
    f.a[i] = *(const u32x4_t*)(sa + row * 128 + ((chunk ^ ((row >> 1) & 7)) << 4));
  }
#pragma unroll
  for (int j = 0; j < 2; ++j) {
    const int row = wn * 64 + j * 32 + lr;
    f.b[j] = *(const u32x4_t*)(sb + row * 128 + ((chunk ^ ((row >> 1) & 7)) << 4));
  }
}
template <int DT, bool RELU_A, bool ZC = false, bool SWAP = false>
__device__ __forceinline__ void pp_mma(PpFrags& f, f32x16_t (&acc)[4][2]) {
#pragma unroll
  for (int i = 0; i < 4; ++i) {
    if (RELU_A) f.a[i] = relu8(f.a[i]);
#pragma unroll
    for (int j = 0; j < 2; ++j) {
      if (ZC) {
        f32x16_t z;
#pragma unroll
        for (int r = 0; r < 16; ++r) z[r] = 0.f;
        acc[i][j] = SWAP ? T16<DT>::mfma32(f.b[j], f.a[i], z) : T16<DT>::mfma32(f.a[i], f.b[j], z);
      } else {
        acc[i][j] = SWAP ? T16<DT>::mfma32(f.b[j], f.a[i], acc[i][j]) : T16<DT>::mfma32(f.a[i], f.b[j], acc[i][j]);
      }
    }
  }
}
template <int DT, bool RELU_A, bool ZC = false, bool SWAP = false>
__device__ __forceinline__ void pp_mma_tile(PpFrags& f0, PpFrags& f1, const char* sa, const char* sb, int wn, int lr, int lh,
                                            f32x16_t (&acc)[4][2]) {
  pp_read(f1, sa, sb, wn, lr, lh, 1);
  __builtin_amdgcn_sched_barrier(0);
  pp_mma<DT, RELU_A, ZC, SWAP>(f0, acc);
  __builtin_amdgcn_sched_barrier(0);
  pp_read(f0, sa, sb, wn, lr, lh, 2);
  __builtin_amdgcn_sched_barrier(0);
  pp_mma<DT, RELU_A, false, SWAP>(f1, acc);
  __builtin_amdgcn_sched_barrier(0);
  pp_read(f1, sa, sb, wn, lr, lh, 3);
  __builtin_amdgcn_sched_barrier(0);
  pp_mma<DT, RELU_A, false, SWAP>(f0, acc);
  __builtin_amdgcn_sched_barrier(0);
  pp_mma<DT, RELU_A, false, SWAP>(f1, acc);
}

template <int DT, int RES>
__device__ __forceinline__ void epilogue_direct(const GemmParams& p, char* smem, int m0, int n0, int wm, int wn, int lr, int lh,
                                                int tid, f32x16_t (&acc)[4][2], bool dma_in_flight, const char* lds_ln) {
  constexpr bool R1 = RES != 0;
  float* sbias = (float*)smem;
  float* scol = sbias + 256;
  float2* lnrow = (float2*)(scol + 256);
  float2* spart = lnrow + 256;
  const bool lnf = p.ln_stats != nullptr;
  u32x4_t rres[4][2][2];
  u32x4_t rnext[2][2][2][2];
  auto row_off = [&](int i) -> long long {
    const int m = m0 + wm * 128 + i * 32 + lr;
    return ((long long)p.c_row_off + (m < p.M ? m : m0)) * p.ldc + n0 + wn * 64 + 8 * lh;
  };
  auto load_next = [&](int i) {
    const long long ro = row_off(i);
#pragma unroll
    for (int j = 0; j < 2; ++j)
#pragma unroll
      for (int pr = 0; pr < 2; ++pr) {
        const long long o = ro + j * 32 + 16 * pr;
        if constexpr (RES == 2) {
          rnext[i & 1][j][pr][0] = *(const u32x4_t*)((const uint16_t*)p.R1 + o);
          rnext[i & 1][j][pr][1] = *(const u32x4_t*)((const uint16_t*)p.R2 + o);
        }
      }
  };
  if constexpr (RES == 1) {
#pragma unroll
    for (int i = 0; i < 4; ++i) {
      const uint16_t* rrow = (const uint16_t*)p.R1 + row_off(i);
#pragma unroll
      for (int j = 0; j < 2; ++j)
#pragma unroll
        for (int pr = 0; pr < 2; ++pr) rres[i][j][pr] = *(const u32x4_t*)(rrow + j * 32 + 16 * pr);
    }
  }
  if constexpr (RES == 2) load_next(0);
  if (tid < 256) {
    sbias[tid] = p.bias != nullptr ? p.bias[n0 + tid] : 0.f;
    scol[tid] = lnf ? p.ln_colsum[n0 + tid] : 0.f;
  } else if (lnf) {
    const int r = tid - 256;
    const bool all8 = p.ln_nblk == 8;
    int m = m0 + r;
    m = m < p.M ? m : m0;
    const float4* st = lds_ln != nullptr ? (const float4*)(lds_ln + r * 64) : (const float4*)(p.ln_stats + (long long)m * 16);
    const float4 r0 = st[0], r1_ = st[1], r2_ = st[2], r3_ = st[3];
    const float sm = (r0.x + r0.z) + (r1_.x + r1_.z) + ((r2_.x + r2_.z) + (all8 ? r3_.x + r3_.z : 0.f));
    const float sq = (r0.y + r0.w) + (r1_.y + r1_.w) + ((r2_.y + r2_.w) + (all8 ? r3_.y + r3_.w : 0.f));
    lnrow[r] = ln_mu_rstd(sm, sq, p.ln_inv_dim, p.ln_eps);
  }
  if (dma_in_flight) asm volatile("s_waitcnt vmcnt(0)" ::: "memory");
  __syncthreads();
  typedef unsigned u32x2_t __attribute__((ext_vector_type(2)));
  const bool stats = R1 && p.row_stats != nullptr;
#pragma unroll
  for (int i = 0; i < 4; ++i) {
    const int row = wm * 128 + i * 32 + lr;
    const int m = m0 + row;
    const bool ok = m < p.M;
    float csm[2][2], csq[2][2];
    if constexpr (RES == 2) {
      if (i + 1 < 4) load_next(i + 1);
    }
    float2 ms = make_float2(0.f, 1.f);
    if (lnf) ms = lnrow[row];
    uint16_t* crow = (uint16_t*)p.C + ((long long)p.c_row_off + (ok ? m : m0)) * p.ldc + n0;
#pragma unroll
    for (int j = 0; j < 2; ++j) {
#pragma unroll
      for (int pr = 0; pr < 2; ++pr) {
        float v[8];
#pragma unroll
        for (int e = 0; e < 4; ++e) {
          const u32x2_t sw = __builtin_amdgcn_permlane32_swap(__float_as_uint(acc[i][j][8 * pr + e]),
                                                              __float_as_uint(acc[i][j][8 * pr + 4 + e]), false, false);
          v[e] = __uint_as_float(sw.x);
          v[4 + e] = __uint_as_float(sw.y);
        }
        const int col = wn * 64 + j * 32 + 8 * (2 * pr + lh);
        const float4 b0 = *(const float4*)(sbias + col), b1 = *(const float4*)(sbias + col + 4);
        const float bb[8] = {b0.x, b0.y, b0.z, b0.w, b1.x, b1.y, b1.z, b1.w};
        if (lnf) {
          const float4 c0 = *(const float4*)(scol + col), c1 = *(const float4*)(scol + col + 4);
          const float cc[8] = {c0.x, c0.y, c0.z, c0.w, c1.x, c1.y, c1.z, c1.w};
#pragma unroll
          for (int e = 0; e < 8; ++e) v[e] = ln_fold_fma(v[e], ms.x, ms.y, cc[e], bb[e]);
        } else {
#pragma unroll
// ... 468 lines not shown
    const int tn_per = tiles_n / p.xcd_n, tm_per = (tiles_m + p.xcd_m - 1) / p.xcd_m;
    const int mt = (x / p.xcd_n) * tm_per + l / tn_per;
    const int nt = (x % p.xcd_n) * tn_per + l % tn_per;
    if (mt >= tiles_m || l >= tm_per * tn_per) return;
    m0 = mt * BM;
    n0 = nt * BN;
  }

  const int kc = tid & 7, r0 = tid >> 3;
  const bool big_m = p.M >= (1 << 23);
  int a_iy0[A_PASSES], a_ix0[A_PASSES];
  long long a_base[A_PASSES];
#pragma unroll
  for (int i = 0; i < A_PASSES; ++i) {
    const int m = m0 + r0 + 32 * i;
    const bool ok = m < p.M;
    const int mm = ok ? m : 0;
    int rem, ox;
    const int img = row_div(mm, p.a_rpi, p.a_rpi_rcp, big_m, rem);
    const int oy = row_div(rem, p.Wout, p.wout_rcp, big_m, ox);
    a_iy0[i] = ok ? oy * p.stride - p.pad_t : -0x40000000;
    a_ix0[i] = ox * p.stride - p.pad_l;
    a_base[i] = (long long)img * p.a_img_stride + p.a_off + ((long long)a_iy0[i] * p.Win + a_ix0[i]) * p.a_pix_stride + kc * 8;
  }
  const char* __restrict__ Ab = (const char*)p.A;
  const uint16_t* __restrict__ Wb = (const uint16_t*)p.W;
  long long w_off[B_PASSES];
#pragma unroll
  for (int j = 0; j < B_PASSES; ++j) w_off[j] = (long long)(n0 + r0 + 32 * j) * p.ldw + kc * 8;

  u32x4_t ra[A_PASSES * A_REGS];
  u32x4_t rb[B_PASSES];
  int ky = 0, kx = 0, c0 = 0;
  const u32x4_t zero4 = {0u, 0u, 0u, 0u};

#define DPTX_LOAD_TILE(K0)                                                                           \
  do {                                                                                               \
    const long long tap_ = (long long)(ky * p.Win + kx) * p.a_pix_stride + c0;                       \
    _Pragma("unroll") for (int i = 0; i < A_PASSES; ++i) {                                           \
      const int iy = a_iy0[i] + ky, ix = a_ix0[i] + kx;                                              \
      const bool valid = ((unsigned)iy < (unsigned)p.Hin) && ((unsigned)ix < (unsigned)p.Win);       \
      const long long e = a_base[i] + tap_;                                                          \
      if constexpr (A_FP32) {                                                                        \
        u32x4_t lo = zero4, hi = zero4;                                                              \
        if (valid) {                                                                                 \
          const u32x4_t* src = (const u32x4_t*)(Ab + e * 4);                                         \
          lo = src[0];                                                                               \
          hi = src[1];                                                                               \
        }                                                                                            \
        ra[2 * i] = lo;                                                                              \
        ra[2 * i + 1] = hi;                                                                          \
      } else {                                                                                       \
        u32x4_t v = zero4;                                                                           \
        if (valid) v = *(const u32x4_t*)(Ab + e * 2);                                                \
        ra[i] = v;                                                                                   \
      }                                                                                              \
    }                                                                                                \
    _Pragma("unroll") for (int j = 0; j < B_PASSES; ++j) rb[j] = *(const u32x4_t*)(Wb + w_off[j] + (K0)); \
    c0 += BK;                                                                                        \
    if (c0 >= p.Cin) {                                                                               \
      c0 = 0;                                                                                        \
      if (++kx == p.ksz) { kx = 0; ++ky; }                                                           \
    }                                                                                                \
  } while (0)

#define DPTX_STORE_TILE(BUF)                                                                         \
  do {                                                                                               \
    char* sa_ = smem + (BUF) * STAGE_BYTES;                                                          \
    char* sb_ = sa_ + BM * 128;                                                                      \
    _Pragma("unroll") for (int i = 0; i < A_PASSES; ++i) {                                           \
      const int row = r0 + 32 * i;                                                                   \
      u32x4_t v;                                                                                     \
      if constexpr (A_FP32) {                                                                        \
        const u32x4_t lo = ra[2 * i], hi = ra[2 * i + 1];                                            \
        v.x = T16<DT>::pack2(__uint_as_float(lo.x), __uint_as_float(lo.y));                          \
        v.y = T16<DT>::pack2(__uint_as_float(lo.z), __uint_as_float(lo.w));                          \
        v.z = T16<DT>::pack2(__uint_as_float(hi.x), __uint_as_float(hi.y));                          \
        v.w = T16<DT>::pack2(__uint_as_float(hi.z), __uint_as_float(hi.w));                          \
      } else {                                                                                       \
        v = ra[i];                                                                                   \
      }                                                                                              \
      if (p.a_relu) v = relu8(v);                                                                    \
      *(u32x4_t*)(sa_ + row * 128 + ((kc ^ ((row >> 1) & 7)) << 4)) = v;                             \
    }                                                                                                \
    _Pragma("unroll") for (int j = 0; j < B_PASSES; ++j) {                                           \
      const int row = r0 + 32 * j;                                                                   \
      *(u32x4_t*)(sb_ + row * 128 + ((kc ^ ((row >> 1) & 7)) << 4)) = rb[j];                         \
    }                                                                                                \
  } while (0)

  f32x16_t acc[TM][TN];
#pragma unroll
  for (int i = 0; i < TM; ++i)
#pragma unroll
    for (int j = 0; j < TN; ++j)
#pragma unroll
      for (int r = 0; r < 16; ++r) acc[i][j][r] = 0.f;

  const int nk = p.K / BK;
  DPTX_LOAD_TILE(0);
  DPTX_STORE_TILE(0);
  __syncthreads();
  for (int kt = 0; kt < nk; ++kt) {
    const bool more = (kt + 1) < nk;
    if (more) DPTX_LOAD_TILE((kt + 1) * BK);
    const char* sa = smem + (kt & 1) * STAGE_BYTES;
    mma_tile<DT, TM, TN, false, 1>(sa, sa + BM * 128, 0, 0, wm, wn, lr, lh, acc);
    if (more) DPTX_STORE_TILE((kt + 1) & 1);
    __syncthreads();
  }
#undef DPTX_LOAD_TILE
#undef DPTX_STORE_TILE
  epilogue<DT, BM, BN, TM, TN>(p, smem, m0, n0, wm, wn, lr, lh, tid, acc);
}

template <int BM, int BN, int PL>
constexpr size_t gemm_smem_bytes() {
  constexpr size_t stage = 2 * (size_t)PL * (BM + BN) * 128;
  constexpr size_t ct_full = (size_t)BM * (BN + 4) * 4;
  constexpr size_t ct = (ct_full > 160 * 1024 ? (size_t)64 * (BN + 4) * 4 : ct_full)
                        + (size_t)BM * 8;
  return stage > ct ? stage : ct;
}

template <typename K>
static void set_smem_attr(K k, size_t smem) { ensure_dyn_smem((const void*)k, smem); }

static void choose_xcd_grid(const GemmParams& p, int tiles_m, int tiles_n, int& xm, int& xn) {
  xm = 8; xn = 1;
  const double a_bytes = (double)p.M * p.K * 2.0, w_bytes = (double)p.N * p.K * 2.0;
  double best = -1.0;
  const int cand[4] = {1, 2, 4, 8};
  for (int c = 0; c < 4; ++c) {
    const int n = cand[c], m = 8 / n;
    if (tiles_n % n != 0 || tiles_m < m) continue;
    const double w_slice = w_bytes / n;
    double cost = n * a_bytes + m * w_bytes;
    if (w_slice > 2.0e6) cost += (double)tiles_m / m * w_slice * 8.0;
    if (best < 0.0 || cost < best) { best = cost; xm = m; xn = n; }
  }
}


template <int DT, int PL, int BM, int BN, int WM_, int WN_, int PLE = PL, int XT = 3>
static hipError_t launch_cfg(const GemmParams& p, hipStream_t stream) {
  const int tiles_m = (p.M + BM - 1) / BM, tiles_n = p.N / BN;
  GemmParams q = p;
  choose_xcd_grid(p, tiles_m, tiles_n, q.xcd_m, q.xcd_n);
  const int tiles = 8 * ((tiles_m + q.xcd_m - 1) / q.xcd_m) * (tiles_n / q.xcd_n);
  constexpr size_t smem = gemm_smem_bytes<BM, BN, PL>();
  const bool glds_ok = !p.a_fp32 && p.a_bytes > 0 && p.a_bytes < (1ll << 31) && (long long)p.N * p.ldw * 2 < (1ll << 31) &&
                       p.M < (1 << 23);
  if (PL == 2 && !glds_ok) return hipErrorInvalidValue;
  if constexpr (DT != DT_FP8 && PL == 1 && BM == 256 && BN == 256) {
    if (glds_ok) {
      constexpr int per_xcd = 32;
      const int grid = tiles / 8 > per_xcd && !(p.debug_flags & 2) ? 8 * per_xcd : tiles;
      constexpr size_t smem_pp = (size_t)256 * 256 + (size_t)8 * 32 * 72 * 4 + (size_t)BM * 8 + (size_t)BM * 64;
      static_assert((size_t)8 * 32 * 72 * 4 >= (size_t)64 * (BN + 4) * 4, "the block-wide slab fits too");
      static_assert(smem_pp >= smem && smem_pp <= 160 * 1024, "stage 0 + the epilogue's slab and row table");
      auto go = [&](auto k) {
        set_smem_attr(k, smem_pp);
        hipLaunchKernelGGL(k, dim3(grid), dim3(512), smem_pp, stream, q);
      };
      const bool direct_any = !(p.debug_flags & 1) && PLE == 1 && !p.bias_per_img && p.c_rpi == 0x7fffffff &&
                              p.C8 == nullptr && p.gn_part == nullptr && p.out_scale == 0.f;
      const bool direct = direct_any && p.R1 == nullptr && p.R2 == nullptr && p.row_stats == nullptr && !p.c_fp32 && p.C16 == nullptr;
      const bool direct_res = direct_any && p.R1 != nullptr && !p.a_relu && p.ln_stats == nullptr;
      const int res = !direct_res ? 0
                      : (!p.r1_fp32 && !p.c_fp32 && p.C16 == nullptr && p.R2 == nullptr) ? 1
                      : (!p.r1_fp32 && !p.c_fp32 && p.C16 == nullptr && p.R2 != nullptr && !p.r2_fp32 && !p.r2_bcast && p.row_stats == nullptr) ? 2
                      : 0;
      if constexpr (PLE == 1) {
        if (direct) {
          if (p.a_relu) go(gemm_pp_kernel<DT, true, 1, 1>);
          else go(gemm_pp_kernel<DT, false, 1, 1>);
          return hipGetLastError();
        }
        if (res == 1) { go(gemm_pp_kernel<DT, false, 1, 2>); return hipGetLastError(); }
        if (res == 2) { go(gemm_pp_kernel<DT, false, 1, 3>); return hipGetLastError(); }
      }
      if (p.a_relu) go(gemm_pp_kernel<DT, true, PLE>);
      else go(gemm_pp_kernel<DT, false, PLE>);
      return hipGetLastError();
    }
  }
  if constexpr (DT != DT_FP8 && PL == 2 && PLE == 2 && BM == 128 && BN == 128 && WM_ == 2 && WN_ == 4) {
    if (!(p.debug_flags & 4) && p.K >= 2 * BK && !p.a_relu) {
      auto k = gemm_pp2_kernel<DT, false, XT>;
      set_smem_attr(k, smem);
      hipLaunchKernelGGL(k, dim3(tiles), dim3(512), smem, stream, q);
      return hipGetLastError();
    }
  }
  if constexpr (DT == DT_FP8) {
    if (!glds_ok || p.a_relu) return hipErrorInvalidValue;
    auto k = gemm_glds_kernel<DT, BM, BN, WM_, WN_, false, PL, PLE>;
    set_smem_attr(k, smem);
    hipLaunchKernelGGL(k, dim3(tiles), dim3(64 * WM_ * WN_), smem, stream, q);
    return hipGetLastError();
  } else
  if (glds_ok) {
    if (p.a_relu) {
      auto k = gemm_glds_kernel<DT, BM, BN, WM_, WN_, true, PL, PLE, XT>;
      set_smem_attr(k, smem);
      hipLaunchKernelGGL(k, dim3(tiles), dim3(64 * WM_ * WN_), smem, stream, q);
    } else {
      auto k = gemm_glds_kernel<DT, BM, BN, WM_, WN_, false, PL, PLE, XT>;
      set_smem_attr(k, smem);
      hipLaunchKernelGGL(k, dim3(tiles), dim3(64 * WM_ * WN_), smem, stream, q);
    }
  } else if constexpr (WM_ * WN_ != 4 || PLE != PL) {
    return hipErrorInvalidValue;
  } else if constexpr (PL == 1) {
    constexpr size_t smem1 = gemm_smem_bytes<BM, BN, 1>();
    if (p.a_fp32) {
      if constexpr (BM == 256) return hipErrorInvalidValue;
      else {
        auto k = gemm_reg_kernel<DT, BM, BN, WM_, WN_, true>;
        set_smem_attr(k, smem1);
        hipLaunchKernelGGL(k, dim3(tiles), dim3(256), smem1, stream, q);
      }
    } else {
      auto k = gemm_reg_kernel<DT, BM, BN, WM_, WN_, false>;
      set_smem_attr(k, smem1);
      hipLaunchKernelGGL(k, dim3(tiles), dim3(256), smem1, stream, q);
    }
  }
  return hipGetLastError();
}

template <int DT, int PL, int PLE = PL, int XT = 3>
static hipError_t launch_dt(const GemmParams& p, hipStream_t stream) {
  const long long m128 = (p.M + 127) / 128, m256 = (p.M + 255) / 256;
  const double sh = p.cu_share > 0.f ? (double)p.cu_share : 1.0;
  const long long cu1 = (long long)(256 * sh + 0.5), cu2 = (long long)(512 * sh + 0.5);
  if constexpr (PL == 1) {
    const bool glds_ok = !p.a_fp32 && p.a_bytes > 0 && p.a_bytes < (1ll << 31) && p.M < (1 << 23);
    if (glds_ok && p.N % 256 == 0 && p.K >= 512) {
      const long long t256 = m256 * (p.N / 256), r256 = (t256 + cu1 - 1) / cu1;
      const long long t128 = m128 * (p.N / 128), r128 = (t128 + cu2 - 1) / cu2;
      const double fill256 = (double)t256 / (double)(r256 * cu1), fill128 = (double)t128 / (double)(r128 * cu2);
      if (t256 >= 200 * sh && fill256 * 1.5 >= fill128) return launch_cfg<DT, PL, 256, 256, 2, 4, PLE, XT>(p, stream);
    }
  }
  if constexpr (PL == 2) {
    if (p.N % 128 == 0 && m128 * (p.N / 128) >= 200) return launch_cfg<DT, PL, 128, 128, 2, 4, PLE, XT>(p, stream);
  }
  if (p.N % 128 == 0 && (m128 * (p.N / 128) >= 256 || p.row_stats != nullptr)) return launch_cfg<DT, PL, 128, 128, 2, 2, PLE, XT>(p, stream);
  if (p.N == 32) return launch_cfg<DT, PL, 256, 32, 4, 1, PLE, XT>(p, stream);
  if (PL == 1 && p.N % 64 == 0 && p.N < 128 && m256 * (p.N / 64) >= 448) return launch_cfg<DT, PL, 256, 64, 4, 1, PLE, XT>(p, stream);
  if (p.N % 64 == 0 && m128 * (p.N / 64) >= 448) return launch_cfg<DT, PL, 128, 64, 2, 2, PLE, XT>(p, stream);
  if (p.N % 64 == 0) return launch_cfg<DT, PL, 64, 64, 2, 2, PLE, XT>(p, stream);
  return hipErrorInvalidValue;
}


hipError_t launch_gemm_16(int dt, const GemmParams& p, hipStream_t stream);
hipError_t launch_gemm_fp16(const GemmParams& p, hipStream_t stream);
hipError_t launch_gemm_fp16e(const GemmParams& p, hipStream_t stream);
hipError_t launch_gemm_x3(int dt, const GemmParams& p, hipStream_t stream);
hipError_t launch_gemm_x2(const GemmParams& p, hipStream_t stream);
hipError_t launch_gemm_fp8(const GemmParams& p, hipStream_t stream);

}
```

### omnidata_amd/csrc/kernels.h

```cpp
#pragma once
#include <hip/hip_runtime.h>
#include <stdint.h>

#include "common.h"

namespace dptx {

void ensure_dyn_smem(const void* kernel, size_t bytes);

struct GemmParams {
  const void* A;
  const void* W;
  void* C;
  const float* bias;
  const void* R1;
  const void* R2;
  int M, N, K;
  int ldw;
  int a_rpi, Wout, Hin, Win, Cin, a_pix_stride;
  long long a_img_stride, a_off;
  long long a_bytes;
  int ksz, stride, pad_t, pad_l;
  int c_rpi, c_img_rows, c_row_off, ldc;
  int r2_bcast;
  int bias_per_img;
  int act;
  int a_relu;
  int a_fp32;
  int c_fp32, r1_fp32, r2_fp32;
  Planes planes;
  int epi2, c_hi_only, r1_hi_only, r2_hi_only;
  int a_hi_only;
  int xcd_m, xcd_n;
  float cu_share;
  float pad0;
  int k_tap_fast;
  float* gn_part;
  int gn_hw, gn_blocks, gn_cpg;
  void* C8;
  int q_relu;
  float out_scale, q_scale;
  const float* out_scale_v;
  void* C16;
  float* row_stats;
  int stats_nblk;
  const float* ln_stats;
  const float* ln_colsum;
  int ln_nblk;
  float ln_eps, ln_inv_dim;
  long long* trace;
  int debug_flags;
  float a_rpi_rcp, wout_rcp;
};

void gemm_params_dense(GemmParams& p, int M, int N, int K);
void gemm_params_conv(GemmParams& p, int B, int Hin, int Win, int Cin, int Cout, int ksz, int stride, int pad_t, int pad_l,
                      int Hout, int Wout, int a_elem_bytes);
hipError_t launch_gemm(int dtype, const GemmParams& p, hipStream_t stream);
void gemm_set_trace(long long* dev_buf);
void gemm_set_debug_flags(int flags);
void gemm_set_cu_share(float share);

hipError_t launch_attention(int mode, const void* qkv, void* out, int B, int S, int heads, Planes pl, hipStream_t stream);

hipError_t launch_layernorm(int mode, const float* x, const float* gamma, const float* beta, void* y,
                            int M, int C, float eps, Planes pl, hipStream_t stream);

struct GnParams {
  const void* X; void* Y;
  const float* gamma; const float* beta;
  float* partial;
  const void* R;
  const float* r_gamma; const float* r_beta; const float* r_partial;
  int B, HW, C, relu;
  float eps;
  int nrec;
};
int gn_chunks(int HW, int C);
hipError_t launch_gn_stats(int mode, const void* X, float* partial, int B, int HW, int C, Planes pl, hipStream_t stream);
hipError_t launch_gn_apply(int mode, const GnParams& p, Planes pl, hipStream_t stream);
hipError_t launch_gn_relu_maxpool(int mode, const void* X, void* Y, const float* gamma, const float* beta,
                                  const float* partial, int B, int H, int W, int C, float eps, Planes pl, hipStream_t stream);

hipError_t launch_stem_conv(int mode, const void* x, int io, const void* Wt, void* y, int B, int H, int W, Planes pl,
                            hipStream_t stream);

hipError_t launch_upsample2x(int mode, const void* X, void* Y, int B, int H, int W, int C, Planes pl, hipStream_t stream,
                             void* Y8 = nullptr, float q_scale = 1.0f, bool out_hi_only = false);
hipError_t launch_amax(int mode, const void* X, size_t n, int relu, unsigned* amax_bits, hipStream_t stream);

hipError_t launch_nonfinite_scan(int mode, const void* X, size_t n, unsigned* flag, hipStream_t stream);

hipError_t launch_checksum(const void* p, size_t bytes, unsigned long long* out, hipStream_t stream);
hipError_t launch_spin(long long ticks_100mhz, hipStream_t stream);

hipError_t launch_head_out(int mode, const void* X, const float* w, const float* b, void* y, int io, int B, int HW,
                           int Cout, int relu, Planes pl, hipStream_t stream);

hipError_t launch_head_tail(int mode, const void* H0, const void* W2, const float* b2, const float* w4, const float* b4,
                            void* y, int io, int B, int Hs, int Ws, int C, int relu_out, hipStream_t stream, Planes pl = Planes{0, 0});
hipError_t launch_pos_resize(const float* src, float* dst, int g_old, int gh, int gw, int C, hipStream_t stream);
hipError_t launch_cls_rows(int mode, const float* cls, const float* pos, float* X, int B, int S, int C, void* X16, float* stats,
                           hipStream_t stream, void* X8 = nullptr, float q_scale = 1.0f);

hipError_t launch_readout_cls(int mode, const float* x, long long x_stride, const void* W, int ldw, int w_off,
                              const float* bias, float* out, int B, int N, int K, Planes pl, hipStream_t stream, int x16 = 0);
hipError_t launch_cast_f32(int mode, const float* src, void* dst, size_t n, Planes pl, hipStream_t stream);

hipError_t launch_patchify16(int mode, const void* x, int io, void* P, int B, int H, int W, Planes pl, hipStream_t stream);
hipError_t launch_depth_to_space(int mode, const void* G, void* Y, int B, int h, int w, int k, int C, Planes pl, hipStream_t stream);

hipError_t launch_to_f32(int mode, const void* src, float* dst, size_t n, Planes pl, hipStream_t stream);

}
```

### omnidata_amd/csrc/norm.hip

```cpp
#include "common.h"
#include "kernels.h"

namespace dptx {

template <int DT, int PL, int VPL>
__global__ __launch_bounds__(256) void layernorm_kernel(const float* __restrict__ x, const float* __restrict__ gamma,
                                                        const float* __restrict__ beta, uint16_t* __restrict__ y,
                                                        int M, int C, float eps, long long plane) {
  const int lane = threadIdx.x & 63;
  const int row = blockIdx.x * 4 + (threadIdx.x >> 6);
  if (row >= M) return;
  const float* xr = x + (long long)row * C;
  float4 v[VPL];
  float s = 0.f;
#pragma unroll
  for (int j = 0; j < VPL; ++j) {
    v[j] = *(const float4*)(xr + (j * 64 + lane) * 4);
    s += (v[j].x + v[j].y) + (v[j].z + v[j].w);
  }
  const float mean = wave_sum(s) / (float)C;
  float q = 0.f;
#pragma unroll
  for (int j = 0; j < VPL; ++j) {
    const float a = v[j].x - mean, b = v[j].y - mean, c = v[j].z - mean, d = v[j].w - mean;
    q += (a * a + b * b) + (c * c + d * d);
  }
  const float rstd = rsqrtf(wave_sum(q) / (float)C + eps);
  uint16_t* yr = y + (long long)row * C;
#pragma unroll
  for (int j = 0; j < VPL; ++j) {
    const int c0 = (j * 64 + lane) * 4;
    const float4 g = *(const float4*)(gamma + c0), bb = *(const float4*)(beta + c0);
    const float o0 = (v[j].x - mean) * rstd * g.x + bb.x, o1 = (v[j].y - mean) * rstd * g.y + bb.y;
    const float o2 = (v[j].z - mean) * rstd * g.z + bb.z, o3 = (v[j].w - mean) * rstd * g.w + bb.w;
    uint2 w;
    w.x = T16<DT>::pack2(o0, o1);
    w.y = T16<DT>::pack2(o2, o3);
    *(uint2*)(yr + c0) = w;
    if (PL == 2) {
      uint2 l;
      l.x = T16<DT>::pack2(o0 - T16<DT>::tof((uint16_t)(w.x & 0xffffu)), o1 - T16<DT>::tof((uint16_t)(w.x >> 16)));
      l.y = T16<DT>::pack2(o2 - T16<DT>::tof((uint16_t)(w.y & 0xffffu)), o3 - T16<DT>::tof((uint16_t)(w.y >> 16)));
      *(uint2*)(yr + plane + c0) = l;
    }
  }
}

hipError_t launch_layernorm(int mode, const float* x, const float* gamma, const float* beta, void* y, int M, int C,
                            float eps, Planes pl, hipStream_t stream) {
  if (C != 768 && C != 1024) return hipErrorInvalidValue;
  dim3 grid((M + 3) / 4);
  if (C == 768) {
    DPTX_DISPATCH_MODE(mode, hipLaunchKernelGGL((layernorm_kernel<DT, PL, 3>), grid, dim3(256), 0, stream, x, gamma, beta,
                                                (uint16_t*)y, M, C, eps, pl.act));
  } else {
    DPTX_DISPATCH_MODE(mode, hipLaunchKernelGGL((layernorm_kernel<DT, PL, 4>), grid, dim3(256), 0, stream, x, gamma, beta,
                                                (uint16_t*)y, M, C, eps, pl.act));
  }
  return hipGetLastError();
}

constexpr int GN_G = 32;

static inline int gn_pix(int C) {
  const int pix = 16384 / C;
  return pix < 16 ? 16 : (pix > 256 ? 256 : pix);
}
int gn_chunks(int HW, int C) {
  const int pix = gn_pix(C);
  return (HW + pix - 1) / pix;
}

template <int DT, int PL>
__global__ __launch_bounds__(256) void gn_stats_kernel(const uint16_t* __restrict__ X, float* __restrict__ partial,
                                                       int HW, int C, int pix, long long plane) {
  __shared__ float red[256 * 8];
  const int tid = threadIdx.x;
  const int cvec = C >> 3;
  const int cpg = C >> 5;
  const int spv = cpg >= 8 ? 1 : 8 / cpg;
  const int v = tid % cvec, p0 = tid / cvec, pstep = 256 / cvec;
  const int b = blockIdx.y, chunk = blockIdx.x;
  const int pbeg = chunk * pix;
  const int pend = min(pbeg + pix, HW);
  float s[4] = {0.f, 0.f, 0.f, 0.f}, q[4] = {0.f, 0.f, 0.f, 0.f};
  const uint16_t* base = X + ((long long)b * HW) * C + v * 8;
  for (int p = pbeg + p0; p < pend; p += pstep) {
    float f[8];
    load8f<DT, PL>(base + (long long)p * C, plane, f);
    if (spv == 1) {
#pragma unroll
      for (int e = 0; e < 8; ++e) { s[0] += f[e]; q[0] += f[e] * f[e]; }
    } else if (spv == 2) {
#pragma unroll
      for (int e = 0; e < 4; ++e) { s[0] += f[e]; q[0] += f[e] * f[e]; s[1] += f[4 + e]; q[1] += f[4 + e] * f[4 + e]; }
    } else {
#pragma unroll
      for (int e = 0; e < 4; ++e) { s[e] += f[2 * e] + f[2 * e + 1]; q[e] += f[2 * e] * f[2 * e] + f[2 * e + 1] * f[2 * e + 1]; }
    }
  }
#pragma unroll
  for (int e = 0; e < 4; ++e) { red[tid * 8 + 2 * e] = s[e]; red[tid * 8 + 2 * e + 1] = q[e]; }
  __syncthreads();
  if (tid < GN_G) {
    const int g = tid;
    int v0, v1, slot;
    if (spv == 1) { v0 = g * (cpg >> 3); v1 = v0 + (cpg >> 3); slot = 0; }
    else { v0 = g / spv; v1 = v0 + 1; slot = g % spv; }
    float ss = 0.f, qq = 0.f;
    for (int pp = 0; pp < pstep; ++pp)
      for (int vv = v0; vv < v1; ++vv) {
        const int t = pp * cvec + vv;
        ss += red[t * 8 + 2 * slot];
        qq += red[t * 8 + 2 * slot + 1];
      }
    float* out = partial + (((long long)b * gridDim.x + chunk) * GN_G + g) * 2;
    out[0] = ss;
    out[1] = qq;
  }
}

hipError_t launch_gn_stats(int mode, const void* X, float* partial, int B, int HW, int C, Planes pl, hipStream_t stream) {
  if (C % 64 != 0 || C > 1024 || (256 % (C / 8)) != 0) return hipErrorInvalidValue;
  dim3 grid(gn_chunks(HW, C), B);
  DPTX_DISPATCH_MODE(mode, hipLaunchKernelGGL((gn_stats_kernel<DT, PL>), grid, dim3(256), 0, stream, (const uint16_t*)X, partial,
                                              HW, C, gn_pix(C), pl.act));
  return hipGetLastError();
}

__device__ __forceinline__ void gn_affine_to_lds(const float* __restrict__ partial, int nchunks, int b,
                                                 const float* __restrict__ gamma, const float* __restrict__ beta, int C,
                                                 int HW, float eps, float* sa, float* sd, float* smr) {
  __shared__ double sred[8][GN_G][2];
  const int tid = threadIdx.x;
  const int cpg = C >> 5;
  {
    const int g = tid & (GN_G - 1), slice = tid >> 5;
    double ss = 0.0, qq = 0.0;
    const float2* pp = (const float2*)partial + (long long)b * nchunks * GN_G + g;
    for (int c = slice; c < nchunks; c += 8) {
      const float2 v = pp[(long long)c * GN_G];
      ss += (double)v.x;
      qq += (double)v.y;
    }
    sred[slice][g][0] = ss;
    sred[slice][g][1] = qq;
  }
  __syncthreads();
  if (tid < GN_G) {
    double ss = 0.0, qq = 0.0;
#pragma unroll
    for (int sl = 0; sl < 8; ++sl) { ss += sred[sl][tid][0]; qq += sred[sl][tid][1]; }
    const double n = (double)HW * (double)cpg;
    const double mean = ss / n;
    double var = qq / n - mean * mean;
    if (var < 0.0) var = 0.0;
    smr[2 * tid] = (float)mean;
    smr[2 * tid + 1] = (float)(1.0 / sqrt(var + (double)eps));
  }
  __syncthreads();
  for (int c = tid; c < C; c += blockDim.x) {
    const int g = c / cpg;
    const float a = smr[2 * g + 1] * gamma[c];
    sa[c] = a;
    sd[c] = beta[c] - smr[2 * g] * a;
  }
  __syncthreads();
}

template <int DT, int PL>
__global__ __launch_bounds__(256) void gn_apply_kernel(const GnParams p, int pix, int nrec, long long plane) {
  __shared__ float sa[1024], sd[1024], ra[1024], rd[1024], smr[64];
  const int b = blockIdx.y;
  gn_affine_to_lds(p.partial, nrec, b, p.gamma, p.beta, p.C, p.HW, p.eps, sa, sd, smr);
  const bool r_gn = (p.R != nullptr) && (p.r_gamma != nullptr);
  if (r_gn) gn_affine_to_lds(p.r_partial, nrec, b, p.r_gamma, p.r_beta, p.C, p.HW, p.eps, ra, rd, smr);
  const int cvec = p.C >> 3;
  const int pbeg = blockIdx.x * pix;
  const int pend = min(pbeg + pix, p.HW);
  const long long img = (long long)b * p.HW * p.C;
  const uint16_t* X = (const uint16_t*)p.X + img;
  const uint16_t* R = p.R ? (const uint16_t*)p.R + img : nullptr;
  uint16_t* Y = (uint16_t*)p.Y + img;
  const int total = (pend - pbeg) * cvec;
  for (int i = threadIdx.x; i < total; i += 256) {
    const int pi = i / cvec, v = i - pi * cvec;
    const long long off = (long long)(pbeg + pi) * p.C + v * 8;
    float f[8];
    load8f<DT, PL>(X + off, plane, f);
#pragma unroll
    for (int e = 0; e < 8; ++e) f[e] = f[e] * sa[v * 8 + e] + sd[v * 8 + e];
    if (R != nullptr) {
      float r[8];
      load8f<DT, PL>(R + off, plane, r);
      if (r_gn) {
#pragma unroll
        for (int e = 0; e < 8; ++e) r[e] = r[e] * ra[v * 8 + e] + rd[v * 8 + e];
      }
#pragma unroll
      for (int e = 0; e < 8; ++e) f[e] += r[e];
    }
    if (p.relu) {
#pragma unroll
      for (int e = 0; e < 8; ++e) f[e] = fmaxf(f[e], 0.f);
    }
    store8f<DT, PL>(Y + off, plane, f);
  }
}

hipError_t launch_gn_apply(int mode, const GnParams& p, Planes pl, hipStream_t stream) {
  if (p.C % 64 != 0 || p.C > 1024) return hipErrorInvalidValue;
  const int nch = gn_chunks(p.HW, p.C);
  const int nrec = p.nrec > 0 ? p.nrec : nch;
  int nb = nch;
  if (p.nrec > 0) {
    int want = 1024 / (p.B > 0 ? p.B : 1);
    want = want < 4 ? 4 : want;
    nb = nch < want ? nch : want;
  }
  const int pix = (p.HW + nb - 1) / nb;
  dim3 grid((p.HW + pix - 1) / pix, p.B);
  DPTX_DISPATCH_MODE(mode, hipLaunchKernelGGL((gn_apply_kernel<DT, PL>), grid, dim3(256), 0, stream, p, pix, nrec, pl.act));
  return hipGetLastError();
}

template <int DT, int PL>
__global__ __launch_bounds__(256) void gn_relu_maxpool_kernel(const uint16_t* __restrict__ X, uint16_t* __restrict__ Y,
                                                              const float* __restrict__ gamma, const float* __restrict__ beta,
                                                              const float* __restrict__ partial, int nchunks, int H, int W,
                                                              int C, float eps, long long plane) {
  __shared__ float sa[1024], sd[1024], smr[64];
  const int b = blockIdx.y;
  gn_affine_to_lds(partial, nchunks, b, gamma, beta, C, H * W, eps, sa, sd, smr);
  const int Ho = (H + 1) / 2, Wo = (W + 1) / 2;
  const int cvec = C >> 3;
  const int total = Ho * Wo * cvec;
  const uint16_t* Xi = X + (long long)b * H * W * C;
  uint16_t* Yo = Y + (long long)b * Ho * Wo * C;
  for (int i = blockIdx.x * 256 + threadIdx.x; i < total; i += gridDim.x * 256) {
    const int v = i % cvec, po = i / cvec;
    const int oy = po / Wo, ox = po - oy * Wo;
    float m[8];
#pragma unroll
    for (int e = 0; e < 8; ++e) m[e] = 0.f;
#pragma unroll
    for (int dy = 0; dy < 3; ++dy) {
      const int iy = 2 * oy + dy;
      if (iy >= H) continue;
#pragma unroll
      for (int dx = 0; dx < 3; ++dx) {
        const int ix = 2 * ox + dx;
        if (ix >= W) continue;
        float f[8];
        load8f<DT, PL>(Xi + ((long long)iy * W + ix) * C + v * 8, plane, f);
#pragma unroll
        for (int e = 0; e < 8; ++e) m[e] = fmaxf(m[e], f[e] * sa[v * 8 + e] + sd[v * 8 + e]);
      }
    }
    store8f<DT, PL>(Yo + (long long)po * C + v * 8, plane, m);
  }
}

hipError_t launch_gn_relu_maxpool(int mode, const void* X, void* Y, const float* gamma, const float* beta,
                                  const float* partial, int B, int H, int W, int C, float eps, Planes pl, hipStream_t stream) {
  if ((H & 1) || (W & 1) || C % 64 != 0 || C > 1024) return hipErrorInvalidValue;
  const int Ho = (H + 1) / 2, Wo = (W + 1) / 2;
  const int total = Ho * Wo * (C / 8);
  dim3 grid(min((total + 255) / 256, 64), B);
  const int nch = gn_chunks(H * W, C);
  DPTX_DISPATCH_MODE(mode, hipLaunchKernelGGL((gn_relu_maxpool_kernel<DT, PL>), grid, dim3(256), 0, stream, (const uint16_t*)X,
                                              (uint16_t*)Y, gamma, beta, partial, nch, H, W, C, eps, pl.act));
  return hipGetLastError();
}

}
```

### omnidata_amd/csrc/ops.hip

```cpp
#include <hip/hip_runtime.h>

#include "../../include/dptx.h"
#include "kernels.h"

using namespace dptx;

extern "C" {

static int rc(hipError_t r) { return r == hipSuccess ? DPTX_OK : DPTX_E_HIP; }

static Planes g_op_planes{0, 0};
int dptx_op_set_planes(int64_t act_plane_elems, int64_t w_plane_elems) {
  g_op_planes.act = act_plane_elems;
  g_op_planes.w = w_plane_elems;
  return DPTX_OK;
}

int dptx_op_gemm(int32_t dtype, const void* A, const void* W, const float* bias, const void* R, void* C, int32_t M, int32_t N,
                 int32_t K, int32_t act, int32_t a_fp32, int32_t c_fp32, int32_t r_fp32, void* stream) {
  GemmParams p;
  gemm_params_dense(p, M, N, K);
  p.A = A; p.W = W; p.C = C; p.bias = bias; p.R1 = R; p.act = act; p.a_fp32 = a_fp32; p.c_fp32 = c_fp32; p.r1_fp32 = r_fp32;
  p.planes = g_op_planes;
  return rc(launch_gemm(dtype, p, (hipStream_t)stream));
}

int dptx_op_gemm_ln(int32_t dtype, const void* A, const void* W, const float* bias, void* C, int32_t M, int32_t N, int32_t K,
                    int32_t act, const float* ln_stats, const float* ln_colsum, int32_t ln_nblk, float ln_eps, void* stream) {
  GemmParams p;
  gemm_params_dense(p, M, N, K);
  p.A = A; p.W = W; p.C = C; p.bias = bias; p.act = act; p.planes = g_op_planes;
  p.ln_stats = ln_stats; p.ln_colsum = ln_colsum; p.ln_nblk = ln_nblk; p.ln_eps = ln_eps; p.ln_inv_dim = 1.0f / (float)K;
  return rc(launch_gemm(dtype, p, (hipStream_t)stream));
}

int dptx_op_gemm_stream(int32_t dtype, const void* A, const void* W, const float* bias, void* C, float* row_stats, int32_t M,
                        int32_t N, int32_t K, void* stream) {
  GemmParams p;
  gemm_params_dense(p, M, N, K);
  p.A = A; p.W = W; p.C = C; p.R1 = C; p.bias = bias; p.planes = g_op_planes;
  p.row_stats = row_stats; p.stats_nblk = 8;
  return rc(launch_gemm(dtype, p, (hipStream_t)stream));
}

int dptx_op_gemm_stream32(int32_t dtype, const void* A, const void* W, const float* bias, float* X, void* C16, float* row_stats,
                          int32_t M, int32_t N, int32_t K, void* stream) {
  GemmParams p;
  gemm_params_dense(p, M, N, K);
  p.A = A; p.W = W; p.C = X; p.c_fp32 = 1; p.R1 = X; p.r1_fp32 = 1; p.C16 = C16; p.bias = bias; p.planes = g_op_planes;
  p.row_stats = row_stats; p.stats_nblk = 8;
  return rc(launch_gemm(dtype, p, (hipStream_t)stream));
}

int dptx_op_head_tail(int32_t dtype, const void* H0, const void* W2, const float* b2, const float* w4, const float* b4, float* y,
                      int32_t B, int32_t Hs, int32_t Ws, int32_t C, int32_t relu_out, void* stream) {
  return rc(launch_head_tail(dtype, H0, W2, b2, w4, b4, y, DPTX_IO_FP32, B, Hs, Ws, C, relu_out, (hipStream_t)stream, g_op_planes));
}

int dptx_op_conv(int32_t dtype, const void* X, const void* Wt, const float* bias, const void* R, void* Y, int32_t B, int32_t H,
                 int32_t W, int32_t Cin, int32_t Cout, int32_t ksize, int32_t stride, int32_t pad_t, int32_t pad_l, int32_t Ho,
                 int32_t Wo, int32_t a_relu, int32_t act, void* stream) {
  GemmParams p;
  gemm_params_conv(p, B, H, W, Cin, Cout, ksize, stride, pad_t, pad_l, Ho, Wo, 2);
  p.A = X; p.W = Wt; p.C = Y; p.bias = bias; p.R1 = R; p.act = act; p.a_relu = a_relu; p.planes = g_op_planes;
  return rc(launch_gemm(dtype, p, (hipStream_t)stream));
}

int dptx_op_conv_planes(int32_t dtype, const void* X, const void* Wt, const float* bias, const void* R, void* Y, int32_t B, int32_t H,
                        int32_t W, int32_t Cin, int32_t Cout, int32_t ksize, int32_t stride, int32_t pad_t, int32_t pad_l, int32_t Ho,
                        int32_t Wo, int32_t a_relu, int32_t act, int32_t epi2, int32_t c_hi_only, int32_t r1_hi_only, void* stream) {
  GemmParams p;
  gemm_params_conv(p, B, H, W, Cin, Cout, ksize, stride, pad_t, pad_l, Ho, Wo, 2);
  p.A = X; p.W = Wt; p.C = Y; p.bias = bias; p.R1 = R; p.act = act; p.a_relu = a_relu; p.planes = g_op_planes;
  p.epi2 = epi2 & 1; p.a_hi_only = (epi2 >> 1) & 1; p.c_hi_only = c_hi_only; p.r1_hi_only = r1_hi_only;
  return rc(launch_gemm(dtype, p, (hipStream_t)stream));
}

int dptx_op_stem_conv(int32_t dtype, const float* x, const void* Wt, void* y, int32_t B, int32_t H, int32_t W, void* stream) {
  return rc(launch_stem_conv(dtype, x, DPTX_IO_FP32, Wt, y, B, H, W, g_op_planes, (hipStream_t)stream));
}

int dptx_op_attention(int32_t dtype, const void* qkv, void* out, int32_t B, int32_t S, int32_t heads, void* stream) {
  return rc(launch_attention(dtype, qkv, out, B, S, heads, g_op_planes, (hipStream_t)stream));
}

int dptx_op_layernorm(int32_t dtype, const float* x, const float* gamma, const float* beta, void* y, int32_t M, int32_t C,
                      float eps, void* stream) {
  return rc(launch_layernorm(dtype, x, gamma, beta, y, M, C, eps, g_op_planes, (hipStream_t)stream));
}

int dptx_op_groupnorm(int32_t dtype, const void* X, const float* gamma, const float* beta, const void* R, void* Y, int32_t B,
                      int32_t HW, int32_t C, int32_t relu, float eps, void* scratch_f32, void* stream) {
  if (scratch_f32 == nullptr) return DPTX_E_INVALID;
  hipError_t r = launch_gn_stats(dtype, X, (float*)scratch_f32, B, HW, C, g_op_planes, (hipStream_t)stream);
  if (r != hipSuccess) return DPTX_E_HIP;
  GnParams g{};
  g.X = X; g.Y = Y; g.gamma = gamma; g.beta = beta; g.partial = (float*)scratch_f32; g.R = R;
  g.B = B; g.HW = HW; g.C = C; g.relu = relu; g.eps = eps;
  return rc(launch_gn_apply(dtype, g, g_op_planes, (hipStream_t)stream));
}

int dptx_op_gn_relu_maxpool(int32_t dtype, const void* X, const float* gamma, const float* beta, void* Y, int32_t B, int32_t H,
                            int32_t W, int32_t C, float eps, void* scratch_f32, void* stream) {
  if (scratch_f32 == nullptr) return DPTX_E_INVALID;
  hipError_t r = launch_gn_stats(dtype, X, (float*)scratch_f32, B, H * W, C, g_op_planes, (hipStream_t)stream);
  if (r != hipSuccess) return DPTX_E_HIP;
  return rc(launch_gn_relu_maxpool(dtype, X, Y, gamma, beta, (const float*)scratch_f32, B, H, W, C, eps, g_op_planes, (hipStream_t)stream));
}

int dptx_op_cls_rows(int32_t dtype, const float* cls, const float* pos, float* X, int32_t B, int32_t S, int32_t C, void* X16,
                     float* row_stats, void* X8, float q_scale, void* stream) {
  if (row_stats != nullptr && C > 8 * 128) return DPTX_E_INVALID;
  return rc(launch_cls_rows(dtype, cls, pos, X, B, S, C, X16, row_stats, (hipStream_t)stream, X8, q_scale));
}

int dptx_debug_set_trace(void* dev_buf) {
  gemm_set_trace((long long*)dev_buf);
  return DPTX_OK;
}

int dptx_debug_set_gemm_flags(int32_t flags) {
  gemm_set_debug_flags(flags);
  return DPTX_OK;
}

int dptx_op_conv_fp8(const void* X8, const void* Wt8, const float* bias, const void* R, void* Y, void* Y8, int32_t B, int32_t H,
                     int32_t W, int32_t Cin, int32_t Cout, int32_t ksize, int32_t stride, int32_t pad_t, int32_t pad_l, int32_t Ho,
                     int32_t Wo, int32_t act, int32_t q_relu, float out_scale, void* stream) {
  GemmParams p;
  gemm_params_conv(p, B, H, W, Cin, Cout, ksize, stride, pad_t, pad_l, Ho, Wo, 1);
  p.A = X8; p.W = Wt8; p.C = Y; p.bias = bias; p.R1 = R; p.C8 = Y8; p.q_relu = q_relu; p.out_scale = out_scale; p.act = act;
  return rc(launch_gemm(MODE_FP8, p, (hipStream_t)stream));
}

int dptx_op_conv_groupnorm(int32_t dtype, const void* X, const void* Wt, void* Yraw, const float* gamma, const float* beta,
                           const void* R, void* Y, int32_t B, int32_t H, int32_t W, int32_t Cin, int32_t Cout, int32_t ksize,
                           int32_t stride, int32_t pad_t, int32_t pad_l, int32_t Ho, int32_t Wo, int32_t relu, float eps,
                           void* scratch_f32, void* stream) {
  if (scratch_f32 == nullptr || (Ho * Wo) % 32 != 0) return DPTX_E_INVALID;
  GemmParams p;
  gemm_params_conv(p, B, H, W, Cin, Cout, ksize, stride, pad_t, pad_l, Ho, Wo, 2);
  p.A = X; p.W = Wt; p.C = Yraw; p.planes = g_op_planes;
  p.gn_part = (float*)scratch_f32; p.gn_hw = Ho * Wo; p.gn_blocks = Ho * Wo / 32; p.gn_cpg = Cout / 32;
  if (launch_gemm(dtype, p, (hipStream_t)stream) != hipSuccess) return DPTX_E_HIP;
  GnParams g{};
  g.X = Yraw; g.Y = Y; g.gamma = gamma; g.beta = beta; g.partial = (float*)scratch_f32; g.R = R;
  g.B = B; g.HW = Ho * Wo; g.C = Cout; g.relu = relu; g.eps = eps; g.nrec = Ho * Wo / 32;
  return rc(launch_gn_apply(dtype, g, g_op_planes, (hipStream_t)stream));
}

int dptx_op_upsample2x(int32_t dtype, const void* X, void* Y, int32_t B, int32_t H, int32_t W, int32_t C, void* stream) {
  return rc(launch_upsample2x(dtype, X, Y, B, H, W, C, g_op_planes, (hipStream_t)stream));
}

}
```

### omnidata_amd/engine.py

```python
from __future__ import annotations

import ctypes as C
import os
from typing import Dict, Optional, Tuple

import numpy as np
import torch

_HERE = os.path.dirname(os.path.abspath(__file__))
LIB_PATH = os.environ.get("DPTX_LIB") or os.path.join(_HERE, "libdptx.so")

DTYPES = {"bf16": 0, "fp16": 1, "bf16x3": 2, "fp16x3": 3, "mixed": 4, "fp8": 5}
TWO_PLANE_DTYPES = frozenset(("bf16x3", "fp16x3", "mixed", "fp8"))
GROUPS = {"resnet": 1, "embed": 2, "vit": 4, "reassemble": 8, "rn": 16, "fusion": 32, "head": 64, "all": 127}
FLAGS = {"no_ln_fold": 1, "group_policy": 2, "fp32_stream": 4, "no_range_check": 8, "fp8_all": 16, "fp8_vit": 32}


def groups_mask(names) -> int:
    if isinstance(names, int):
        return names
    if isinstance(names, str):
        names = [n for n in names.replace(",", "+").split("+") if n]
    mask = 0
    for n in names:
        mask |= GROUPS[n]
    return mask


BACKBONE_IDS = {"vitb_rn50_384": 0, "vitl16_384": 1}
ERRORS = {0: "ok", -1: "invalid argument / call order", -2: "state_dict key error", -3: "HIP error",
          -4: "no device", -5: "allocation failed"}


class DptxConfig(C.Structure):
    _fields_ = [("num_channels", C.c_int32), ("max_batch", C.c_int32), ("dtype", C.c_int32),
                ("device_id", C.c_int32), ("non_negative", C.c_int32), ("ws_form", C.c_int32),
                ("ws_eps", C.c_float), ("max_height", C.c_int32), ("max_width", C.c_int32),
                ("dual_task", C.c_int32), ("streams", C.c_int32), ("x3_groups", C.c_int32), ("backbone", C.c_int32),
                ("flags", C.c_int32), ("reserved", C.c_int32)]


_vp, _i32, _i64p, _f32p, _sz = C.c_void_p, C.c_int32, C.POINTER(C.c_int64), C.POINTER(C.c_float), C.c_size_t
ABI = [
    ("dptx_default_config", None, [C.POINTER(DptxConfig)]),
    ("dptx_create", C.c_int, [C.POINTER(_vp), C.POINTER(DptxConfig)]),
    ("dptx_destroy", None, [_vp]),
    ("dptx_load_tensor", C.c_int, [_vp, C.c_char_p, _vp, _i64p, _i32]),
    ("dptx_finalize_weights", C.c_int, [_vp]),
    ("dptx_packed_bytes", _sz, [_vp]),
    ("dptx_export_packed_host", C.c_int, [_vp, _vp, _sz]),
    ("dptx_export_packed_device", C.c_int, [_vp, _vp, _sz, _vp]),
    ("dptx_import_packed_device", C.c_int, [_vp, _vp, _sz, _vp]),
    ("dptx_workspace_bytes", _sz, [_vp]),
    ("dptx_forward", C.c_int, [_vp, _vp, _i32, _vp, _i32, _vp]),
    ("dptx_forward_hw", C.c_int, [_vp, _vp, _i32, _vp, _i32, _i32, _i32, _vp]),
    ("dptx_forward_dual", C.c_int, [_vp, _vp, _i32, _vp, _vp, _i32, _i32, _i32, _vp]),
    ("dptx_set_layer_precision", C.c_int, [_vp, C.c_char_p, _i32]),
    ("dptx_tune_schedule", C.c_int, [_vp, _vp, _i32, _vp, _vp, _i32, _i32, _i32, _i32, _vp]),
    ("dptx_schedule_info", C.c_int, [_vp, C.POINTER(C.c_int32), C.POINTER(C.c_int32), _f32p, _f32p]),
    ("dptx_probe_stream_overlap", C.c_int, [_i32, _vp, _vp, _i32, _f32p]),
    ("dptx_calibrate_fp8", C.c_int, [_vp, _vp, _i32, _vp, _vp, _i32, _i32, _i32, _vp]),
    ("dptx_fp8_get_calibration", C.c_int, [_vp, _f32p, _f32p, _i32]),
    ("dptx_share_packed", C.c_int, [_vp, _vp]),
    ("dptx_fp8_set_calibration", C.c_int, [_vp, _f32p, _i32]),
    ("dptx_range_status", C.c_int, [_vp, C.POINTER(C.c_int32), _i32, _vp]),
    ("dptx_tap", C.c_int, [_vp, C.c_char_p, _vp, _sz, _i64p]),
    ("dptx_enable_taps", C.c_int, [_vp, C.c_int]),
    ("dptx_forward_info", C.c_int, [_vp, _i64p, C.POINTER(C.c_double), C.POINTER(C.c_double)]),
    ("dptx_set_profiling", C.c_int, [_vp, C.c_int]),
    ("dptx_profile_get", C.c_int, [_vp, _i32, C.POINTER(C.c_double), _i64p, C.POINTER(C.c_double)]),
    ("dptx_profile_dump", C.c_int, [_vp, C.c_char_p]),
    ("dptx_last_error", C.c_char_p, [_vp]),
    ("dptx_version", C.c_char_p, []),
    ("dptx_preprocess_u8", C.c_int, [_vp, _i32, _i32, _i32, _i32, _i32, _vp, _vp]),
    ("dptx_postprocess_normal_u8", C.c_int, [_vp, _vp, _vp]),
    ("dptx_postprocess_depth", C.c_int, [_vp, _vp, _vp]),
    ("dptx_resample_coeffs", C.c_int, [_i32, _i32, C.POINTER(C.c_int32), C.POINTER(C.c_int32), _i32, C.POINTER(C.c_int32)]),
    ("dptx_refocus_workspace_bytes", C.c_int, [_i32, _i32, _i32, _i32, _i32, _i64p]),
    ("dptx_refocus_quantiles", C.c_int, [_vp, _i32, _i32, _i32, _i32, _vp, _vp, C.c_int64, _vp]),
    ("dptx_refocus", C.c_int, [_vp, _vp, _i32, _i32, _i32, _i32, _i32, _vp, _vp, _vp, _vp, _vp, _vp, C.c_int64, _vp]),
    ("dptx_midas_workspace_bytes", C.c_int, [_i32, _i32, _i32, _i32, _i64p]),
    ("dptx_midas_loss", C.c_int, [_vp, _vp, _vp, _i32, _i32, _i32, _i32, _i32, _i32, C.c_float, _vp, _vp, _vp, C.c_int64, _vp]),
    ("dptx_midas_loss_backward", C.c_int, [_vp, _vp, _vp, _i32, _i32, _i32, _i32, _i32, _i32, C.c_float, _vp, _vp, _vp, _vp]),
    ("dptx_midas_stats", C.c_int, [_vp, _vp, _vp, _i32, _i32, _i32, _i32, _vp, _vp, _vp, _vp, C.c_int64, _vp]),
    ("dptx_vnl_workspace_bytes", C.c_int, [_i32, _i32, _i32, _i32, _i64p]),
    ("dptx_vnl_prepare", C.c_int, [_vp, _vp, _vp, _i32, _i32, _i32, _vp, _vp, C.c_int64, _vp]),
    ("dptx_vnl_loss", C.c_int, [_vp, _vp, _i32, _i32, _i32, C.c_float, C.c_float, C.c_float, _vp, _vp, _vp, _i32, _i32, _vp, _vp,
                                _vp, C.c_int64, _vp]),
    ("dptx_vnl_loss_backward", C.c_int, [_vp, _vp, _i32, _i32, _i32, C.c_float, C.c_float, _vp, _vp, _vp, _i32, _vp, _vp, _vp, _vp,
                                         _vp, _vp]),
    ("dptx_vnl_triples", C.c_int, [_vp, _vp, _i32, _i32, _i32, C.c_float, C.c_float, C.c_float, _vp, _vp, _vp, _i32, _vp, _vp, _vp,
                                   _vp]),
    ("dptx_normal_workspace_bytes", C.c_int, [_i32, _i32, _i32, _i64p]),
    ("dptx_normal_loss", C.c_int, [_vp, _vp, _vp, _i32, _i32, _i32, _i32, C.c_float, _vp, _vp, _vp, C.c_int64, _vp]),
    ("dptx_normal_loss_backward", C.c_int, [_vp, _vp, _vp, _i32, _i32, _i32, _i32, C.c_float, _vp, _vp, _vp, _vp]),
    ("dptx_normal_pixels", C.c_int, [_vp, _vp, _vp, _i32, _i32, _i32, _i32, _vp, _vp, _vp]),
    ("dptx_masked_workspace_bytes", C.c_int, [C.c_int64, _i64p]),
    ("dptx_masked_loss", C.c_int, [_vp, _vp, _vp, C.c_int64, _i32, _vp, _vp, _vp, C.c_int64, _vp]),
    ("dptx_masked_loss_backward", C.c_int, [_vp, _vp, _vp, C.c_int64, _i32, _vp, _vp, _vp, _vp]),
    ("dptx_valid_mask", C.c_int, [_vp, _i32, _i32, _i32, _i32, _vp, _vp]),
    ("dptx_eval_workspace_bytes", C.c_int, [_i32, _i32, _i32, _i64p]),
    ("dptx_eval_normal", C.c_int, [_vp, _vp, _vp, _i32, _i32, _i32, _i32, _vp, _vp, C.c_int64, _vp]),
    ("dptx_eval_depth", C.c_int, [_vp, _vp, _vp, _i32, _i32, _i32, _i32, _vp, _vp, C.c_int64, _vp]),
    ("dptx_eval_normal_pixels", C.c_int, [_vp, _vp, _i32, _i32, _i32, _vp, _vp]),
    ("dptx_op_set_planes", C.c_int, [C.c_int64, C.c_int64]),
    ("dptx_op_gemm", C.c_int, [_i32, _vp, _vp, _vp, _vp, _vp, _i32, _i32, _i32, _i32, _i32, _i32, _i32, _vp]),
    ("dptx_op_conv", C.c_int, [_i32, _vp, _vp, _vp, _vp, _vp] + [_i32] * 13 + [_vp]),
    ("dptx_op_conv_planes", C.c_int, [_i32, _vp, _vp, _vp, _vp, _vp] + [_i32] * 16 + [_vp]),
    ("dptx_op_stem_conv", C.c_int, [_i32, _vp, _vp, _vp, _i32, _i32, _i32, _vp]),
    ("dptx_op_attention", C.c_int, [_i32, _vp, _vp, _i32, _i32, _i32, _vp]),
    ("dptx_op_layernorm", C.c_int, [_i32, _vp, _vp, _vp, _vp, _i32, _i32, C.c_float, _vp]),
    ("dptx_op_groupnorm", C.c_int, [_i32, _vp, _vp, _vp, _vp, _vp, _i32, _i32, _i32, _i32, C.c_float, _vp, _vp]),
    ("dptx_op_gn_relu_maxpool", C.c_int, [_i32, _vp, _vp, _vp, _vp, _i32, _i32, _i32, _i32, C.c_float, _vp, _vp]),
    ("dptx_op_cls_rows", C.c_int, [_i32, _vp, _vp, _vp, _i32, _i32, _i32, _vp, _vp, _vp, C.c_float, _vp]),
    ("dptx_debug_set_trace", C.c_int, [_vp]),
    ("dptx_debug_set_gemm_flags", C.c_int, [C.c_int32]),
    ("dptx_debug_arena_fill", C.c_int, [_vp, _i32]),
    ("dptx_debug_arena_read", C.c_int, [_vp, _vp, _sz, _sz]),
    ("dptx_debug_arena_layout", C.c_int, [_vp, C.c_char_p, _sz]),
    ("dptx_debug_arena_checksums", C.c_int, [_vp, _vp, _i32, _vp]),
    ("dptx_op_conv_fp8", C.c_int, [_vp, _vp, _vp, _vp, _vp, _vp] + [_i32] * 13 + [C.c_float, _vp]),
    ("dptx_op_conv_groupnorm", C.c_int, [_i32, _vp, _vp, _vp, _vp, _vp, _vp, _vp] + [_i32] * 12 + [C.c_float, _vp, _vp]),
    ("dptx_op_upsample2x", C.c_int, [_i32, _vp, _vp, _i32, _i32, _i32, _i32, _vp]),
    ("dptx_op_gemm_ln", C.c_int, [_i32, _vp, _vp, _vp, _vp, _i32, _i32, _i32, _i32, _vp, _vp, _i32, C.c_float, _vp]),
    ("dptx_op_gemm_stream", C.c_int, [_i32, _vp, _vp, _vp, _vp, _vp, _i32, _i32, _i32, _vp]),
    ("dptx_op_gemm_stream32", C.c_int, [_i32, _vp, _vp, _vp, _vp, _vp, _vp, _i32, _i32, _i32, _vp]),
    ("dptx_op_head_tail", C.c_int, [_i32, _vp, _vp, _vp, _vp, _vp, _vp, _i32, _i32, _i32, _i32, _i32, _vp]),
]

_lib = None


def _embedded_hash(path: str) -> str:
    import re
    try:
        with open(path, "rb") as f:
            data = f.read()
    except OSError:
        return ""
    m = re.search(rb"dptx [0-9.]+ \(gfx950[^)]*\) src=([0-9a-f]{16})", data)
    return m.group(1).decode() if m else ""


def load_library() -> C.CDLL:
    global _lib
    if _lib is None:
        check = not os.environ.get("DPTX_LIB") and not os.environ.get("DPTX_SKIP_HASH_CHECK")
        want = ""
        if check:
            from .build import build, source_hash
            want = source_hash(os.environ.get("DPTX_CXXFLAGS", "").split())
            have = _embedded_hash(LIB_PATH) if os.path.exists(LIB_PATH) else ""
            if have != want:
                hipcc = os.environ.get("HIPCC", "/opt/rocm/bin/hipcc")
                if not os.path.exists(hipcc):
                    raise RuntimeError(f"{LIB_PATH} is {'stale (built from sources ' + have + ')' if have else 'missing'}; the tree "
                                       f"has {want} and {hipcc} is not available: run `python -m omnidata_amd.build` on a "
                                       "machine with ROCm. There is no CPU fallback.")
                build()
        if not os.path.exists(LIB_PATH):
            raise RuntimeError(f"{LIB_PATH} not found: run `python -m omnidata_amd.build` "
                               "(or __graft_entry__.build()). There is no CPU fallback.")
        lib = C.CDLL(LIB_PATH)
        for name, res, args in ABI:
            fn = getattr(lib, name)
            fn.restype = res
            fn.argtypes = args
        if check:
            built = lib.dptx_version().decode().rsplit("src=", 1)[-1]
            if built != want:
                raise RuntimeError(f"{LIB_PATH} is stale: built from sources {built}, the tree has {want}. "
                                   "Run `python -m omnidata_amd.build --force`.")
        _lib = lib
    return _lib


def _ptr(t) -> int:
    return 0 if t is None else t.data_ptr()


def _stream(device=None) -> int:
    return torch.cuda.current_stream(device).cuda_stream


IO_DTYPES = {torch.float32: 0, torch.bfloat16: 1, torch.float16: 2}


def probe_stream_overlap(stream_a, stream_b, device_index: int = 0, spin_us: int = 2000) -> float:
    r = C.c_float(0)
    rc = load_library().dptx_probe_stream_overlap(int(device_index), stream_a.cuda_stream, stream_b.cuda_stream, int(spin_us), C.byref(r))
    if rc != 0:
        raise RuntimeError(f"dptx_probe_stream_overlap failed: {ERRORS.get(rc, rc)}")
    return float(r.value)


def check_image_shape(x: torch.Tensor):
    if x.dim() != 4 or x.shape[1] != 3 or x.shape[2] % 32 or x.shape[3] % 32:
        raise ValueError(f"expected [B,3,H,W] with H, W multiples of 32 (384x384 is the trained size), got {tuple(x.shape)}")


class Engine:

    def __init__(self, num_channels: int = 3, max_batch: int = 32, dtype: str = "mixed",
                 device_id: Optional[int] = 0, non_negative: bool = True, ws_form: int = 0, ws_eps: float = 1e-8,
                 max_hw: Tuple[int, int] = (384, 384), dual: bool = False, streams: int = 0, x3_groups=0,
                 backbone: str = "vitb_rn50_384", flags: int = 0):
        self.lib = load_library()
        cfg = DptxConfig()
        self.lib.dptx_default_config(C.byref(cfg))
        cfg.num_channels, cfg.max_batch, cfg.dtype = num_channels, max_batch, DTYPES[dtype]
        cfg.device_id = -1 if device_id is None else int(device_id)
        cfg.non_negative, cfg.ws_form, cfg.ws_eps = int(non_negative), ws_form, ws_eps
        cfg.max_height, cfg.max_width = int(max_hw[0]), int(max_hw[1])
        cfg.dual_task = int(dual)
        cfg.streams = int(streams)
        cfg.x3_groups = groups_mask(x3_groups)
        cfg.backbone = BACKBONE_IDS[backbone]
        cfg.flags = int(flags)
        self.cfg = cfg
        self.fp8_calibrated = False
        self.fp8_scales = None
        self.layer_precision: Dict[str, int] = {}
        self._schedule_tuned = bool(streams) or bool(os.environ.get("DPTX_STREAMS")) or device_id is None
        self.dtype = dtype
        self.backbone = backbone
        self.h = _vp()
        rc = self.lib.dptx_create(C.byref(self.h), C.byref(cfg))
        if rc != 0:
            self.h = None
            raise RuntimeError(f"dptx_create failed: {ERRORS.get(rc, rc)}"
                               + (" (no HIP device visible; the HIP path has no CPU fallback)" if rc == -4 else ""))

    def _check(self, rc: int, what: str):
        if rc != 0:
            msg = self.lib.dptx_last_error(self.h).decode()
            raise RuntimeError(f"{what} failed ({ERRORS.get(rc, rc)}): {msg}")

    def close(self):
        if getattr(self, "h", None):
            self.lib.dptx_destroy(self.h)
            self.h = None

    def __del__(self):
        try:
            self.close()
        except Exception:
            pass

    def config_kwargs(self) -> dict:
        c = self.cfg
        return dict(num_channels=c.num_channels, max_batch=c.max_batch, dtype=self.dtype,
                    device_id=None if c.device_id < 0 else c.device_id, non_negative=bool(c.non_negative), ws_form=c.ws_form,
                    ws_eps=c.ws_eps, max_hw=(c.max_height, c.max_width), dual=bool(c.dual_task), streams=c.streams,
                    x3_groups=c.x3_groups, backbone=self.backbone, flags=c.flags)

    def follow(self, owner: "Engine"):
        self.share_weights_from(owner)
        self.copy_layer_precision_from(owner)
        if owner.fp8_scales is not None:
            self.set_fp8_calibration(owner.fp8_scales)

    def load_state_dict(self, sd: Dict[str, torch.Tensor]):
        for k, v in sd.items():
            a = v.detach().to("cpu", torch.float32).contiguous().numpy()
            shape = (C.c_int64 * a.ndim)(*a.shape)
            self._check(self.lib.dptx_load_tensor(self.h, k.encode(), a.ctypes.data, shape, a.ndim), f"load_tensor({k})")
        self._check(self.lib.dptx_finalize_weights(self.h), "finalize_weights")

    @property
    def packed_bytes(self) -> int:
        return self.lib.dptx_packed_bytes(self.h)

    @property
    def workspace_bytes(self) -> int:
# ... 211 lines not shown
```

Before: 2694 images/s.

## Fuse GroupNorm+ReLU into the A-operand prologue of ResNet bottleneck convs

In the ResNet bottleneck blocks, the standalone GroupNorm-apply passes after conv1 and conv2 are removed. The next convolution now normalizes its A tiles on the fly. Each GEMM block computes the per-image GroupNorm scale and shift into LDS from the partial statistics, then applies the affine transform, ReLU and a padding mask to each A fragment before the MFMA. This drops two full read-write passes over the activations per block. The cost is extra ALU work per fragment, more LDS use, and a restricted tile configuration, which may lower GEMM efficiency.

Result: slower. 2473 images/s (-8.2%).

```diff
diff --git a/include/dptx.h b/include/dptx.h
--- a/include/dptx.h
+++ b/include/dptx.h
@@ -230,6 +230,9 @@
                            const void* R, void* Y, int32_t B, int32_t H, int32_t W, int32_t Cin, int32_t Cout,
                            int32_t ksize, int32_t stride, int32_t pad_t, int32_t pad_l, int32_t Ho, int32_t Wo,
                            int32_t relu, float eps, void* scratch_f32, void* stream);
+int dptx_op_conv_gn_a(int32_t dtype, const void* Xraw, const float* records, const float* gamma, const float* beta, float eps,
+                      const void* Wt, void* Y, int32_t B, int32_t H, int32_t W, int32_t Cin, int32_t Cout, int32_t ksize,
+                      int32_t stride, int32_t pad_t, int32_t pad_l, int32_t Ho, int32_t Wo, void* gn_out_scratch, void* stream);
 int dptx_op_upsample2x(int32_t dtype, const void* X, void* Y, int32_t B, int32_t H, int32_t W,
                        int32_t C, void* stream);
 int dptx_op_gemm_ln(int32_t dtype, const void* A, const void* W, const float* bias, void* C, int32_t M, int32_t N, int32_t K,
diff --git a/omnidata_amd/build.py b/omnidata_amd/build.py
--- a/omnidata_amd/build.py
+++ b/omnidata_amd/build.py
@@ -8,7 +8,7 @@
 CSRC = os.path.join(HERE, "csrc")
 LIB = os.path.join(HERE, "libdptx.so")
 SOURCES = ["gemm.hip", "gemm_fp16.hip", "gemm_fp16e.hip", "gemm_x3.hip", "gemm_x2.hip", "gemm_fp8.hip", "attention.hip", "norm.hip", "misc.hip", "stem.hip", "head.hip", "prepost.hip", "refocus.hip", "midas_loss.hip", "vnl_loss.hip", "normal_loss.hip", "eval_metrics.hip", "engine.hip", "ops.hip"]
-HEADERS = ["common.h", "kernels.h", "gemm_impl.h", "select.h", os.path.join("..", "..", "include", "dptx.h")]
+HEADERS = ["common.h", "kernels.h", "gemm_impl.h", "gn_affine.h", "select.h", os.path.join("..", "..", "include", "dptx.h")]
 _NOPK = ["-Xclang", "-target-feature", "-Xclang", "-packed-fp32-ops"]
 SOURCE_FLAGS = {src: list(_NOPK) for src in ("norm.hip", "misc.hip", "gemm.hip", "gemm_fp16.hip", "gemm_fp16e.hip", "gemm_x3.hip",
                                              "gemm_x2.hip", "gemm_fp8.hip", "refocus.hip",
diff --git a/omnidata_amd/csrc/engine.hip b/omnidata_amd/csrc/engine.hip
--- a/omnidata_amd/csrc/engine.hip
+++ b/omnidata_amd/csrc/engine.hip
@@ -664,6 +664,9 @@
   const void *R1_ = nullptr, *R2_ = nullptr;
   int q_ = 0;
   float* gn_part_ = nullptr;
+  const float* gna_part_ = nullptr;
+  const char* gna_key_ = nullptr;
+  float* gna_ad_ = nullptr;
   int out_lo_ = -1;
   int c_fp32_ = 0, r1_fp32_ = 0;
   int ln_ = LN_NONE;
@@ -675,6 +678,7 @@
   GemmOpt& R2(const void* v) { R2_ = v; return *this; }
   GemmOpt& q(int v) { q_ = v; return *this; }
   GemmOpt& gn_part(float* v) { gn_part_ = v; return *this; }
+  GemmOpt& gn_a(const float* part, const char* key, float* ad) { gna_part_ = part; gna_key_ = key; gna_ad_ = ad; return *this; }
   GemmOpt& out_lo(int v) { out_lo_ = v; return *this; }
   GemmOpt& c_fp32(int v) { c_fp32_ = v; return *this; }
   GemmOpt& r1_fp32(int v) { r1_fp32_ = v; return *this; }
@@ -760,6 +764,15 @@
     }
     p.act = o.act_; p.a_relu = o.a_relu_; p.planes = e->pl;
     if (o.gn_part_) { p.gn_part = o.gn_part_; p.gn_hw = Hout * Wout; p.gn_blocks = Hout * Wout / 32; p.gn_cpg = Cout / 32; }
+    if (o.gna_part_) {
+      const std::string nkey = o.gna_key_;
+      p.gna_part = o.gna_part_; p.gna_gamma = e->f(nkey + ".weight"); p.gna_beta = e->f(nkey + ".bias");
+      p.gna_hw = Hin * Win; p.gna_blocks = Hin * Win / 32; p.gna_eps = 1e-5f;
+      if (o.gna_ad_) {
+        chk(launch_gn_affine(p.gna_part, p.gna_blocks, p.gna_gamma, p.gna_beta, o.gna_ad_, B, p.gna_hw, Cin, p.gna_eps, st), o.gna_key_, 2);
+        p.gna_ad = o.gna_ad_;
+      }
+    }
     if (f8) {
       p.A = e->q8(in); p.W = e->w8(wkey); p.a_relu = 0;
       p.out_scale = 1.0f / q8_scale_of(in); p.out_scale_v = e->wscale(wkey);
@@ -783,6 +796,17 @@
   }
 
   static bool gn_fusable(int HW) { return HW % 32 == 0; }
+  enum { GNA_PASS = 0, GNA_PROLOGUE = 1, GNA_TABLE = 2 };
+#ifndef DPTX_GNA_MODES
+#define DPTX_GNA_MODES {GNA_PROLOGUE, GNA_PROLOGUE, GNA_PROLOGUE}
+#endif
+  int gna_mode(int stage, int HWin, int HWout, int C) const {
+    static const int modes[3] = DPTX_GNA_MODES;
+    const bool single = dt == MODE_BF16 || dt == MODE_FP16;
+    if (!single || e->mixed() || e->fp8() || (gemm_get_debug_flags() & 8) || !gn_fusable(HWin) || HWout < 256 || C > 256) return GNA_PASS;
+    if ((long long)B * HWin * C * 2 >= (1ll << 31) || (long long)B * HWout >= (1 << 23)) return GNA_PASS;
+    return modes[stage];
+  }
   void gn_stats(const void* X, float* part, int HW, int C) { chk(launch_gn_stats(dt, X, part, B, HW, C, e->pl, st), "gn_stats", 2); }
   void gn_apply(void* X, const std::string& nkey, float* part, int HW, int C, int relu, const void* R = nullptr,
                 const std::string& rkey = "", const float* rpart = nullptr) {
@@ -863,12 +887,17 @@
       }
       conv(cur, H, Wd, cin, p + "conv1.weight", 1, 1, 0, 0, H, Wd, mid, A(E->T1), GemmOpt().gn_part(f_in ? part0 : nullptr));
       if (!f_in) gn_stats(A(E->T1), part0, H * Wd, mid);
-      gn_apply(A(E->T1), p + "norm1", part0, H * Wd, mid, 1);
+      const int g1 = gna_mode(s, H * Wd, Ho * Wo, mid), g2 = gna_mode(s, Ho * Wo, Ho * Wo, mid);
+      const std::string n1 = p + "norm1", n2 = p + "norm2";
+      GemmOpt o2 = GemmOpt().gn_part(f_out ? part1 : nullptr), o3 = GemmOpt().gn_part(f_out ? part2 : nullptr);
+      if (g1 != GNA_PASS) o2.gn_a(part0, n1.c_str(), g1 == GNA_TABLE ? part0 + (size_t)B * (H * Wd / 32) * 64 : nullptr);
+      else gn_apply(A(E->T1), n1, part0, H * Wd, mid, 1);
       const int pad = (stride == 1) ? 1 : 0;
-      conv(A(E->T1), H, Wd, mid, p + "conv2.weight", 3, stride, pad, pad, Ho, Wo, mid, A(E->T2), GemmOpt().gn_part(f_out ? part1 : nullptr));
+      conv(A(E->T1), H, Wd, mid, p + "conv2.weight", 3, stride, pad, pad, Ho, Wo, mid, A(E->T2), o2);
       if (!f_out) gn_stats(A(E->T2), part1, Ho * Wo, mid);
-      gn_apply(A(E->T2), p + "norm2", part1, Ho * Wo, mid, 1);
-      conv(A(E->T2), Ho, Wo, mid, p + "conv3.weight", 1, 1, 0, 0, Ho, Wo, cout, out, GemmOpt().gn_part(f_out ? part2 : nullptr));
+      if (g2 != GNA_PASS) o3.gn_a(part1, n2.c_str(), g2 == GNA_TABLE ? part1 + (size_t)B * (Ho * Wo / 32) * 64 : nullptr);
+      else gn_apply(A(E->T2), n2, part1, Ho * Wo, mid, 1);
+      conv(A(E->T2), Ho, Wo, mid, p + "conv3.weight", 1, 1, 0, 0, Ho, Wo, cout, out, o3);
       if (!f_out) gn_stats(out, part2, Ho * Wo, cout);
       if (b == 0)
         gn_apply(out, p + "norm3", part2, Ho * Wo, cout, 1, A(E->DS), p + "downsample.norm", part3);
diff --git a/omnidata_amd/csrc/gemm.hip b/omnidata_amd/csrc/gemm.hip
--- a/omnidata_amd/csrc/gemm.hip
+++ b/omnidata_amd/csrc/gemm.hip
@@ -30,6 +30,7 @@
 void gemm_set_trace(long long* dev_buf) { g_trace = dev_buf; }
 static thread_local int g_debug_flags = 0;
 void gemm_set_debug_flags(int flags) { g_debug_flags = flags; }
+int gemm_get_debug_flags() { return g_debug_flags; }
 static thread_local float g_cu_share = 1.0f;
 void gemm_set_cu_share(float share) { g_cu_share = share > 0.f && share <= 1.f ? share : 1.0f; }
 
@@ -47,6 +48,9 @@
   if (p.ln_stats != nullptr && (p.R1 != nullptr || p.R2 != nullptr || p.bias_per_img || p.ln_colsum == nullptr || (p.ln_nblk != 6 && p.ln_nblk != 8) ||
                                 p.c_rpi != 0x7fffffff || p.gn_part != nullptr))
     return hipErrorInvalidValue;
+  if (p.gna_part != nullptr && (mode == MODE_FP8 || p.epi2 || p.a_relu || p.a_fp32 || p.k_tap_fast || p.Cin > 256 || p.ksz > 3 ||
+                                p.gna_hw % 32 != 0 || p.gna_blocks != p.gna_hw / 32 || p.gna_gamma == nullptr || p.gna_beta == nullptr))
+    return hipErrorInvalidValue;
   if (mode == MODE_FP8) {
     if (p.K % 128 != 0 || p.Cin % 128 != 0 || p.M <= 0 || p.N % 32 != 0 || p.ldw < p.K || p.ldw % 16 != 0 || p.gn_part != nullptr)
       return hipErrorInvalidValue;
diff --git a/omnidata_amd/csrc/gemm_impl.h b/omnidata_amd/csrc/gemm_impl.h
--- a/omnidata_amd/csrc/gemm_impl.h
+++ b/omnidata_amd/csrc/gemm_impl.h
@@ -3,6 +3,7 @@
 #include <type_traits>
 
 #include "common.h"
+#include "gn_affine.h"
 #include "kernels.h"
 
 namespace dptx {
@@ -37,9 +38,19 @@
   return t;
 }
 
-template <int DT, int TM, int TN, bool RELU_A, int PL = 1, int HK = BK / 16, int XT = 3>
+constexpr int GNA_C = 256;
+constexpr int GNA_LDS = 4 * GNA_C * 4 + 2 * GN_G * 4;
+struct GnaTile {
+  const float* tab = nullptr;
+  bool one_img = true;
+  unsigned sel = 0;
+  unsigned ok = 0;
+};
+
+template <int DT, int TM, int TN, bool RELU_A, int PL = 1, int HK = BK / 16, int XT = 3, bool GN_A = false>
 __device__ __forceinline__ void mma_tile(const char* sa, const char* sb, int a_lo, int b_lo, int wm, int wn, int lr, int lh,
-                                         f32x16_t (&acc)[TM][TN]) {
+                                         f32x16_t (&acc)[TM][TN], const GnaTile& gna = GnaTile()) {
+  static_assert(!GN_A || (PL == 1 && DT != DT_FP8 && !RELU_A), "GroupNorm on the A path: one 16-bit plane, no pre-activation");
   if constexpr (DT == DT_FP8) {
     static_assert(PL == 1 && !RELU_A, "fp8: single plane; the producer writes the ReLU'd copy");
     typedef int i32x8_t __attribute__((ext_vector_type(8)));
@@ -74,6 +85,17 @@
 #pragma unroll
     for (int g = 0; g < BK / 16; g += HK) {
       u32x4_t af[HK][TM], bf[HK][TN];
+      float4 ga[GN_A ? HK : 1][2] = {}, gd[GN_A ? HK : 1][2] = {};
+      if constexpr (GN_A) {
+        if (gna.one_img) {
+#pragma unroll
+          for (int ks = 0; ks < HK; ++ks) {
+            const float* t = gna.tab + (2 * (g + ks) + lh) * 8;
+            ga[ks][0] = *(const float4*)t; ga[ks][1] = *(const float4*)(t + 4);
+            gd[ks][0] = *(const float4*)(t + GNA_C); gd[ks][1] = *(const float4*)(t + GNA_C + 4);
+          }
+        }
+      }
 #pragma unroll
       for (int ks = 0; ks < HK; ++ks) {
         const int chunk = 2 * (g + ks) + lh;
@@ -94,6 +116,19 @@
 #pragma unroll
         for (int i = 0; i < TM; ++i) {
           if (RELU_A) af[ks][i] = relu8(af[ks][i]);
+          if constexpr (GN_A) {
+            float4 a0 = ga[ks][0], a1 = ga[ks][1], d0 = gd[ks][0], d1 = gd[ks][1];
+            if (!gna.one_img) {
+              const float* t = gna.tab + (2 * (g + ks) + lh) * 8 + ((gna.sel >> i) & 1u) * (2 * GNA_C);
+              a0 = *(const float4*)t; a1 = *(const float4*)(t + 4);
+              d0 = *(const float4*)(t + GNA_C); d1 = *(const float4*)(t + GNA_C + 4);
+            }
+            uint4 x;
+            x.x = af[ks][i].x; x.y = af[ks][i].y; x.z = af[ks][i].z; x.w = af[ks][i].w;
+            x = gn_affine_relu8<DT>(x, a0, a1, d0, d1);
+            const unsigned keep = ((gna.ok >> i) & 1u) ? 0xffffffffu : 0u;
+            af[ks][i] = u32x4_t{x.x & keep, x.y & keep, x.z & keep, x.w & keep};
+          }
 #pragma unroll
           for (int j = 0; j < TN; ++j) acc[i][j] = T16<DT>::mfma32(af[ks][i], bf[ks][j], acc[i][j]);
         }
@@ -452,7 +487,7 @@
 
 constexpr unsigned OOB = 0x80000000u;
 
-template <int DT, int BM, int BN, int WAVES_M, int WAVES_N, bool RELU_A, int PL, int PLE = PL, int XT = 3>
+template <int DT, int BM, int BN, int WAVES_M, int WAVES_N, bool RELU_A, int PL, int PLE = PL, int XT = 3, bool GN_A = false>
 __global__ __launch_bounds__(64 * WAVES_M * WAVES_N, PL == 2 ? 1 : 2) void gemm_glds_kernel(const GemmParams p) {
 #if defined(__HIP_DEVICE_COMPILE__)
   constexpr int NT = 64 * WAVES_M * WAVES_N;
@@ -519,6 +554,37 @@
       (void*)((uint16_t*)const_cast<void*>(p.W) + (PL == 2 ? p.planes.w : 0)), 0, w_bytes, 0x00020000);
 
   int ky = 0, kx = 0, c0 = 0;
+
+  static_assert(!GN_A || (NT == 256 && PL == 1 && PLE == 1), "GroupNorm on the A path: 4-wave single-plane tiles");
+  float* const gna_tab = (float*)(smem + 2 * STAGE_BYTES);
+  unsigned gna_mask[TM];
+  GnaTile gna;
+  int gna_img0 = 0, gna_img1 = 0, gna_tap = 0, gna_c0 = 0;
+  if constexpr (GN_A) {
+    const int last = (m0 + BM < p.M ? m0 + BM : p.M) - 1;
+    gna_img0 = m0 / p.a_rpi;
+    gna_img1 = last / p.a_rpi;
+    gna.one_img = gna_img1 == gna_img0;
+#pragma unroll
+    for (int i = 0; i < TM; ++i) {
+      const int m = m0 + wm * (TM * 32) + i * 32 + lr;
+      unsigned mask = 0;
+      if (m < p.M) {
+        int rem, ox;
+        const int img = row_div(m, p.a_rpi, p.a_rpi_rcp, false, rem);
+        const int oy = row_div(rem, p.Wout, p.wout_rcp, false, ox);
+        const int iy0 = oy * p.stride - p.pad_t, ix0 = ox * p.stride - p.pad_l;
+#pragma unroll
+        for (int t = 0; t < 9; ++t) {
+          const int ty = t / 3, tx = t % 3;
+          if (ty < p.ksz && tx < p.ksz && (unsigned)(iy0 + ty) < (unsigned)p.Hin && (unsigned)(ix0 + tx) < (unsigned)p.Win)
+            mask |= 1u << (ty * p.ksz + tx);
+        }
+        gna.sel |= (img != gna_img0 ? 1u : 0u) << i;
+      }
+      gna_mask[i] = mask;
+    }
+  }
 
 #define DPTX_ISSUE_TILE(BUF, K0)                                                                                   \
   do {                                                                                                             \
@@ -577,6 +643,22 @@
   if (tr && wave == 0) { trp[62 * 4 + 0] = (long long)__builtin_readcyclecounter(); trp[62 * 4 + 1] = (long long)wall_clock64(); }
 #endif
   DPTX_ISSUE_TILE(0, 0);
+  if constexpr (GN_A) {
+    float* smr = gna_tab + 4 * GNA_C;
+    if (p.gna_ad != nullptr) {
+      for (int c = tid; c < 2 * p.Cin; c += NT) {
+        const int h = c >= p.Cin ? 1 : 0, cc = c - h * p.Cin;
+        gna_tab[h * GNA_C + cc] = p.gna_ad[(long long)gna_img0 * 2 * p.Cin + c];
+        gna_tab[(2 + h) * GNA_C + cc] = p.gna_ad[(long long)gna_img1 * 2 * p.Cin + c];
+      }
+    } else {
+      gn_affine_to_lds(p.gna_part, p.gna_blocks, gna_img0, p.gna_gamma, p.gna_beta, p.Cin, p.gna_hw, p.gna_eps, gna_tab,
+                       gna_tab + GNA_C, smr);
+      if (!gna.one_img)
+        gn_affine_to_lds(p.gna_part, p.gna_blocks, gna_img1, p.gna_gamma, p.gna_beta, p.Cin, p.gna_hw, p.gna_eps,
+                         gna_tab + 2 * GNA_C, gna_tab + 3 * GNA_C, smr);
+    }
+  }
   for (int kt = 0; kt < nk; ++kt) {
     asm volatile("s_waitcnt vmcnt(0)" ::: "memory");
     DPTX_STAMP(3);
@@ -585,7 +667,15 @@
     const char* sa = smem + (kt & 1) * STAGE_BYTES;
     if (kt + 1 < nk) DPTX_ISSUE_TILE((kt + 1) & 1, (kt + 1) * BK);
     DPTX_STAMP(1);
-    mma_tile<DT, TM, TN, RELU_A, PL, HK, XT>(sa, sa + B_BASE, A_LO, B_LO, wm, wn, lr, lh, acc);
+    if constexpr (GN_A) {
+      gna.tab = gna_tab + gna_c0;
+      gna.ok = 0;
+#pragma unroll
+      for (int i = 0; i < TM; ++i) gna.ok |= ((gna_mask[i] >> gna_tap) & 1u) << i;
+      gna_c0 += BK;
+      if (gna_c0 >= p.Cin) { gna_c0 = 0; ++gna_tap; }
+    }
+    mma_tile<DT, TM, TN, RELU_A, PL, HK, XT, GN_A>(sa, sa + B_BASE, A_LO, B_LO, wm, wn, lr, lh, acc, gna);
     DPTX_STAMP(2);
   }
 #ifdef DPTX_TRACE
@@ -1360,6 +1450,20 @@
   const bool glds_ok = !p.a_fp32 && p.a_bytes > 0 && p.a_bytes < (1ll << 31) && (long long)p.N * p.ldw * 2 < (1ll << 31) &&
                        p.M < (1 << 23);
   if (PL == 2 && !glds_ok) return hipErrorInvalidValue;
+  if (p.gna_part != nullptr) {
+    if constexpr (DT != DT_FP8 && PL == 1 && PLE == 1 && WM_ == 2 && WN_ == 2) {
+      if (!glds_ok || p.a_relu || p.k_tap_fast || p.Cin > GNA_C || p.ksz > 3 || p.a_rpi < BM) return hipErrorInvalidValue;
+      constexpr size_t stages = 2 * (size_t)(BM + BN) * 128 + GNA_LDS;
+      constexpr size_t smem_g = stages > smem ? stages : smem;
+      static_assert(smem_g + sizeof(double) * 8 * GN_G * 2 <= 80 * 1024, "two blocks per CU");
+      auto k = gemm_glds_kernel<DT, BM, BN, WM_, WN_, false, 1, 1, 3, true>;
+      set_smem_attr(k, smem_g);
+      hipLaunchKernelGGL(k, dim3(tiles), dim3(256), smem_g, stream, q);
+      return hipGetLastError();
+    } else {
+      return hipErrorInvalidValue;
+    }
+  }
   if constexpr (DT != DT_FP8 && PL == 1 && BM == 256 && BN == 256) {
     if (glds_ok) {
       constexpr int per_xcd = 32;
@@ -1443,6 +1547,14 @@
   const long long m128 = (p.M + 127) / 128, m256 = (p.M + 255) / 256;
   const double sh = p.cu_share > 0.f ? (double)p.cu_share : 1.0;
   const long long cu1 = (long long)(256 * sh + 0.5), cu2 = (long long)(512 * sh + 0.5);
+  if (p.gna_part != nullptr) {
+    if constexpr (DT != DT_FP8 && PL == 1 && PLE == 1) {
+      if (p.N % 128 == 0 && m128 * (p.N / 128) >= 256) return launch_cfg<DT, 1, 128, 128, 2, 2, 1, XT>(p, stream);
+      if (p.N % 64 == 0 && m128 * (p.N / 64) >= 448) return launch_cfg<DT, 1, 128, 64, 2, 2, 1, XT>(p, stream);
+      if (p.N % 64 == 0) return launch_cfg<DT, 1, 64, 64, 2, 2, 1, XT>(p, stream);
+    }
+    return hipErrorInvalidValue;
+  }
   if constexpr (PL == 1) {
     const bool glds_ok = !p.a_fp32 && p.a_bytes > 0 && p.a_bytes < (1ll << 31) && p.M < (1 << 23);
     if (glds_ok && p.N % 256 == 0 && p.K >= 512) {
diff --git a/omnidata_amd/csrc/gn_affine.h b/omnidata_amd/csrc/gn_affine.h
--- /dev/null
+++ b/omnidata_amd/csrc/gn_affine.h
@@ -0,0 +1,60 @@
+#pragma once
+#include "common.h"
+
+namespace dptx {
+
+constexpr int GN_G = 32;
+
+__device__ __forceinline__ void gn_affine_to_lds(const float* __restrict__ partial, int nchunks, int b,
+                                                 const float* __restrict__ gamma, const float* __restrict__ beta, int C,
+                                                 int HW, float eps, float* sa, float* sd, float* smr) {
+  __shared__ double sred[8][GN_G][2];
+  const int tid = threadIdx.x;
+  const int cpg = C >> 5;
+  {
+    const int g = tid & (GN_G - 1), slice = tid >> 5;
+    double ss = 0.0, qq = 0.0;
+    const float2* pp = (const float2*)partial + (long long)b * nchunks * GN_G + g;
+    for (int c = slice; c < nchunks; c += 8) {
+      const float2 v = pp[(long long)c * GN_G];
+      ss += (double)v.x;
+      qq += (double)v.y;
+    }
+    sred[slice][g][0] = ss;
+    sred[slice][g][1] = qq;
+  }
+  __syncthreads();
+  if (tid < GN_G) {
+    double ss = 0.0, qq = 0.0;
+#pragma unroll
+    for (int sl = 0; sl < 8; ++sl) { ss += sred[sl][tid][0]; qq += sred[sl][tid][1]; }
+    const double n = (double)HW * (double)cpg;
+    const double mean = ss / n;
+    double var = qq / n - mean * mean;
+    if (var < 0.0) var = 0.0;
+    smr[2 * tid] = (float)mean;
+    smr[2 * tid + 1] = (float)(1.0 / sqrt(var + (double)eps));
+  }
+  __syncthreads();
+  for (int c = tid; c < C; c += blockDim.x) {
+    const int g = c / cpg;
+    const float a = smr[2 * g + 1] * gamma[c];
+    sa[c] = a;
+    sd[c] = beta[c] - smr[2 * g] * a;
+  }
+  __syncthreads();
+}
+
+template <int DT>
+__device__ __forceinline__ uint4 gn_affine_relu8(const uint4& x, const float4& a0, const float4& a1, const float4& d0,
+                                                 const float4& d1) {
+  float f[8];
+  unpack8<DT>(x, f);
+  f[0] = fmaxf(fmaf(f[0], a0.x, d0.x), 0.f); f[1] = fmaxf(fmaf(f[1], a0.y, d0.y), 0.f);
+  f[2] = fmaxf(fmaf(f[2], a0.z, d0.z), 0.f); f[3] = fmaxf(fmaf(f[3], a0.w, d0.w), 0.f);
+  f[4] = fmaxf(fmaf(f[4], a1.x, d1.x), 0.f); f[5] = fmaxf(fmaf(f[5], a1.y, d1.y), 0.f);
+  f[6] = fmaxf(fmaf(f[6], a1.z, d1.z), 0.f); f[7] = fmaxf(fmaf(f[7], a1.w, d1.w), 0.f);
+  return pack8<DT>(f);
+}
+
+}
diff --git a/omnidata_amd/csrc/kernels.h b/omnidata_amd/csrc/kernels.h
--- a/omnidata_amd/csrc/kernels.h
+++ b/omnidata_amd/csrc/kernels.h
@@ -51,6 +51,12 @@
   long long* trace;
   int debug_flags;
   float a_rpi_rcp, wout_rcp;
+  const float* gna_part;
+  const float* gna_gamma;
+  const float* gna_beta;
+  const float* gna_ad;
+  int gna_hw, gna_blocks;
+  float gna_eps;
 };
 
 void gemm_params_dense(GemmParams& p, int M, int N, int K);
@@ -59,6 +65,7 @@
 hipError_t launch_gemm(int dtype, const GemmParams& p, hipStream_t stream);
 void gemm_set_trace(long long* dev_buf);
 void gemm_set_debug_flags(int flags);
+int gemm_get_debug_flags();
 void gemm_set_cu_share(float share);
 
 hipError_t launch_attention(int mode, const void* qkv, void* out, int B, int S, int heads, Planes pl, hipStream_t stream);
@@ -79,6 +86,8 @@
 int gn_chunks(int HW, int C);
 hipError_t launch_gn_stats(int mode, const void* X, float* partial, int B, int HW, int C, Planes pl, hipStream_t stream);
 hipError_t launch_gn_apply(int mode, const GnParams& p, Planes pl, hipStream_t stream);
+hipError_t launch_gn_affine(const float* partial, int nrec, const float* gamma, const float* beta, float* ad, int B, int HW,
+                            int C, float eps, hipStream_t stream);
 hipError_t launch_gn_relu_maxpool(int mode, const void* X, void* Y, const float* gamma, const float* beta,
                                   const float* partial, int B, int H, int W, int C, float eps, Planes pl, hipStream_t stream);
 
diff --git a/omnidata_amd/csrc/norm.hip b/omnidata_amd/csrc/norm.hip
--- a/omnidata_amd/csrc/norm.hip
+++ b/omnidata_amd/csrc/norm.hip
@@ -1,4 +1,5 @@
 #include "common.h"
+#include "gn_affine.h"
 #include "kernels.h"
 
 namespace dptx {
@@ -60,7 +61,6 @@
   return hipGetLastError();
 }
 
-constexpr int GN_G = 32;
 
 static inline int gn_pix(int C) {
   const int pix = 16384 / C;
@@ -126,46 +126,6 @@
   DPTX_DISPATCH_MODE(mode, hipLaunchKernelGGL((gn_stats_kernel<DT, PL>), grid, dim3(256), 0, stream, (const uint16_t*)X, partial,
                                               HW, C, gn_pix(C), pl.act));
   return hipGetLastError();
-}
-
-__device__ __forceinline__ void gn_affine_to_lds(const float* __restrict__ partial, int nchunks, int b,
-                                                 const float* __restrict__ gamma, const float* __restrict__ beta, int C,
-                                                 int HW, float eps, float* sa, float* sd, float* smr) {
-  __shared__ double sred[8][GN_G][2];
-  const int tid = threadIdx.x;
-  const int cpg = C >> 5;
-  {
-    const int g = tid & (GN_G - 1), slice = tid >> 5;
-    double ss = 0.0, qq = 0.0;
-    const float2* pp = (const float2*)partial + (long long)b * nchunks * GN_G + g;
-    for (int c = slice; c < nchunks; c += 8) {
-      const float2 v = pp[(long long)c * GN_G];
-      ss += (double)v.x;
-      qq += (double)v.y;
-    }
-    sred[slice][g][0] = ss;
-    sred[slice][g][1] = qq;
-  }
-  __syncthreads();
-  if (tid < GN_G) {
-    double ss = 0.0, qq = 0.0;
-#pragma unroll
-    for (int sl = 0; sl < 8; ++sl) { ss += sred[sl][tid][0]; qq += sred[sl][tid][1]; }
-    const double n = (double)HW * (double)cpg;
-    const double mean = ss / n;
-    double var = qq / n - mean * mean;
-    if (var < 0.0) var = 0.0;
-    smr[2 * tid] = (float)mean;
-    smr[2 * tid + 1] = (float)(1.0 / sqrt(var + (double)eps));
-  }
-  __syncthreads();
-  for (int c = tid; c < C; c += blockDim.x) {
-    const int g = c / cpg;
-    const float a = smr[2 * g + 1] * gamma[c];
-    sa[c] = a;
-    sd[c] = beta[c] - smr[2 * g] * a;
-  }
-  __syncthreads();
 }
 
 template <int DT, int PL>
@@ -189,7 +149,7 @@
     float f[8];
     load8f<DT, PL>(X + off, plane, f);
 #pragma unroll
-    for (int e = 0; e < 8; ++e) f[e] = f[e] * sa[v * 8 + e] + sd[v * 8 + e];
+    for (int e = 0; e < 8; ++e) f[e] = fmaf(f[e], sa[v * 8 + e], sd[v * 8 + e]);
     if (R != nullptr) {
       float r[8];
       load8f<DT, PL>(R + off, plane, r);
@@ -221,6 +181,25 @@
   const int pix = (p.HW + nb - 1) / nb;
   dim3 grid((p.HW + pix - 1) / pix, p.B);
   DPTX_DISPATCH_MODE(mode, hipLaunchKernelGGL((gn_apply_kernel<DT, PL>), grid, dim3(256), 0, stream, p, pix, nrec, pl.act));
+  return hipGetLastError();
+}
+
+__global__ __launch_bounds__(256) void gn_affine_kernel(const float* __restrict__ partial, int nrec, const float* __restrict__ gamma,
+                                                        const float* __restrict__ beta, float* __restrict__ ad, int HW, int C,
+                                                        float eps) {
+  __shared__ float sa[1024], sd[1024], smr[64];
+  const int b = blockIdx.x;
+  gn_affine_to_lds(partial, nrec, b, gamma, beta, C, HW, eps, sa, sd, smr);
+  for (int c = threadIdx.x; c < C; c += 256) {
+    ad[(long long)b * 2 * C + c] = sa[c];
+    ad[(long long)b * 2 * C + C + c] = sd[c];
+  }
+}
+
+hipError_t launch_gn_affine(const float* partial, int nrec, const float* gamma, const float* beta, float* ad, int B, int HW,
+                            int C, float eps, hipStream_t stream) {
+  if (C % 64 != 0 || C > 1024 || nrec <= 0) return hipErrorInvalidValue;
+  hipLaunchKernelGGL(gn_affine_kernel, dim3(B), dim3(256), 0, stream, partial, nrec, gamma, beta, ad, HW, C, eps);
   return hipGetLastError();
 }
 
diff --git a/omnidata_amd/csrc/ops.hip b/omnidata_amd/csrc/ops.hip
--- a/omnidata_amd/csrc/ops.hip
+++ b/omnidata_amd/csrc/ops.hip
@@ -149,6 +149,21 @@
   return rc(launch_gn_apply(dtype, g, g_op_planes, (hipStream_t)stream));
 }
 
+int dptx_op_conv_gn_a(int32_t dtype, const void* Xraw, const float* records, const float* gamma, const float* beta, float eps,
+                      const void* Wt, void* Y, int32_t B, int32_t H, int32_t W, int32_t Cin, int32_t Cout, int32_t ksize,
+                      int32_t stride, int32_t pad_t, int32_t pad_l, int32_t Ho, int32_t Wo, void* gn_out_scratch, void* stream) {
+  if (records == nullptr || gamma == nullptr || beta == nullptr || (H * W) % 32 != 0) return DPTX_E_INVALID;
+  if (gn_out_scratch != nullptr && (Ho * Wo) % 32 != 0) return DPTX_E_INVALID;
+  GemmParams p;
+  gemm_params_conv(p, B, H, W, Cin, Cout, ksize, stride, pad_t, pad_l, Ho, Wo, 2);
+  p.A = Xraw; p.W = Wt; p.C = Y; p.planes = g_op_planes;
+  p.gna_part = records; p.gna_gamma = gamma; p.gna_beta = beta; p.gna_hw = H * W; p.gna_blocks = H * W / 32; p.gna_eps = eps;
+  if (gn_out_scratch != nullptr) {
+    p.gn_part = (float*)gn_out_scratch; p.gn_hw = Ho * Wo; p.gn_blocks = Ho * Wo / 32; p.gn_cpg = Cout / 32;
+  }
+  return rc(launch_gemm(dtype, p, (hipStream_t)stream));
+}
+
 int dptx_op_upsample2x(int32_t dtype, const void* X, void* Y, int32_t B, int32_t H, int32_t W, int32_t C, void* stream) {
   return rc(launch_upsample2x(dtype, X, Y, B, H, W, C, g_op_planes, (hipStream_t)stream));
 }
diff --git a/omnidata_amd/engine.py b/omnidata_amd/engine.py
--- a/omnidata_amd/engine.py
+++ b/omnidata_amd/engine.py
@@ -120,6 +120,7 @@
     ("dptx_debug_arena_layout", C.c_int, [_vp, C.c_char_p, _sz]),
     ("dptx_debug_arena_checksums", C.c_int, [_vp, _vp, _i32, _vp]),
     ("dptx_op_conv_fp8", C.c_int, [_vp, _vp, _vp, _vp, _vp, _vp] + [_i32] * 13 + [C.c_float, _vp]),
+    ("dptx_op_conv_gn_a", C.c_int, [_i32, _vp, _vp, _vp, _vp, C.c_float, _vp, _vp] + [_i32] * 11 + [_vp, _vp]),
     ("dptx_op_conv_groupnorm", C.c_int, [_i32, _vp, _vp, _vp, _vp, _vp, _vp, _vp] + [_i32] * 12 + [C.c_float, _vp, _vp]),
     ("dptx_op_upsample2x", C.c_int, [_i32, _vp, _vp, _i32, _i32, _i32, _i32, _vp]),
     ("dptx_op_gemm_ln", C.c_int, [_i32, _vp, _vp, _vp, _vp, _i32, _i32, _i32, _i32, _vp, _vp, _i32, C.c_float, _vp]),
```
